# olegiy/manuscript-ocr

Measured on AMD Instinct MI355X. Metric: manuscript pages/sec end-to-end (EAST+TRBA) at 1/2/4/8 MI355X; CER vs CPU ref, higher is better.
Workload: dtype f32 (bf16x3 split operands on the 1x1 / Winograd-domain GEMMs, f32 accumulate)

## Files before the change

### include/msocr.h

```cpp
#ifndef MSOCR_H
#define MSOCR_H
#include <stdint.h>

#ifdef __cplusplus
extern "C" {
#endif

#define MSOCR_F32 0
#define MSOCR_BF16 1

#define MSOCR_OK 0
#define MSOCR_E_ARG (-1)
#define MSOCR_E_LAUNCH (-2)
#define MSOCR_E_NOGPU (-3)

#define MSOCR_CONV_RELU 1u
#define MSOCR_CONV_RESIDUAL 2u
#define MSOCR_CONV_POOL2 4u

typedef struct msocr_conv_desc {
  int32_t dtype;
  int32_t N, H, W, Cin;
  int64_t in_sN, in_sH, in_sW;
  int32_t KH, KW, stride_h, stride_w, pad_h, pad_w;
  int32_t Ho, Wo, Cout;
  int64_t out_ld;
  int64_t res_ld;
  uint32_t flags;
} msocr_conv_desc;

int msocr_conv2d(const msocr_conv_desc* d, const void* in, const void* weight, const float* bias,
                 const void* residual, void* out, void* stream);

#define MSOCR_WINO_2X2 0
#define MSOCR_WINO_4X2 1
#define MSOCR_WINO_4X4 2
int64_t msocr_winograd_workspace_bytes(const msocr_conv_desc* d, int form);
int msocr_winograd_weights_host(int form, const float* w_khwc_host, int Cout, int Cin, float* u_out_host);
int msocr_conv3x3_winograd(const msocr_conv_desc* d, int form, int split, const void* in, const void* u, const float* bias,
                           const void* residual, void* out, void* workspace, void* stream);
int msocr_winograd_input_transform(const msocr_conv_desc* d, int form, const void* in, void* workspace, void* stream);
int msocr_winograd_gemm(const msocr_conv_desc* d, int form, int split, const void* u, void* workspace, void* stream);
int msocr_winograd_output_transform(const msocr_conv_desc* d, int form, const void* workspace, const float* bias, const void* residual,
                                    void* out, void* stream);

int msocr_split_bf16x3_host(const float* w_host, int64_t n, uint16_t* planes_out_host);
int msocr_split_bf16x3_ktile_host(const float* w_host, int64_t nbatch, int64_t rows, int64_t k, uint16_t* planes_out_host);
int msocr_conv1x1_split(const msocr_conv_desc* d, const void* in, const void* weight_planes, const float* bias,
                        const void* residual, void* out, void* stream);
int msocr_conv2d_split(const msocr_conv_desc* d, const void* in, const void* weight_planes, const float* bias,
                       const void* residual, void* out, void* stream);

int64_t msocr_winograd_fused64_workspace_bytes(const msocr_conv_desc* d);
int msocr_conv3x3_winograd_fused64(const msocr_conv_desc* d, int split, const void* in, const void* u, const float* bias,
                                   const void* residual, void* out, void* workspace, void* stream);
int msocr_winograd_fused64_gemm_output(const msocr_conv_desc* d, int split, const void* u, const void* workspace, const float* bias,
                                       const void* residual, void* out, void* stream);

int msocr_normalize_u8(const uint8_t* src, int N, int H, int W, int pad_t, int pad_l, int Hp, int Wp, int cpad,
                       int mode, int dtype, void* out, void* stream);

int msocr_resize_linear_u8(const uint8_t* src, int N, int sh, int sw, uint8_t* dst, int dh, int dw, void* stream);

int msocr_maxpool2d(const void* in, int N, int H, int W, int C, int64_t in_ld, int k, int s, int p, int dtype,
                    void* out, int Ho, int Wo, int64_t out_ld, void* stream);

int msocr_upsample2x_bilinear(const void* in, int N, int H, int W, int C, int64_t in_ld, int dtype, void* out,
                              int64_t out_ld, void* stream);

int msocr_east_head(const void* h1, int64_t npix, int64_t in_ld, int dtype, const float* w9, const float* b9,
                    float* score_out, float* geo_out, void* stream);

int msocr_east_decode(const float* score, const float* geo, int N, int H, int W, float thresh, float scale,
                      int quant, float* cand_out, int32_t* count_out, int max_cand, void* stream);

int64_t msocr_lanms_workspace_bytes(int N, int max_cand);
int msocr_east_lanms(const float* cand, const int32_t* counts, int N, int max_cand, double iou_thr, float* boxes_out,
                     int32_t* nbox_out, void* workspace, void* stream);

int64_t msocr_east_box_tail_workspace_bytes(int N, int max_cand);
int msocr_east_box_tail(const float* boxes, const int32_t* nbox, int N, int max_cand, double expand_w, double expand_h,
                        double scale_x, double scale_y, int axis_aligned_output, int remove_anomalies, double sigma, int min_count,
                        float* out, int32_t* n_out, void* workspace, void* stream);
int msocr_east_box_tail_host(const float* quads_host, int M, double expand_w, double expand_h, double scale_x, double scale_y,
                             int axis_aligned_output, int remove_anomalies, double sigma, int min_count, float* out_host,
                             int32_t* n_out_host);


int msocr_se_residual(const void* x, const void* identity, int N, int HW, int C, int dtype, const float* w1,
                      const float* w2, float* gate_ws, void* out, void* stream);

int msocr_mean_over_h(const void* in, int N, int H, int W, int C, int dtype, float* out, void* stream);

int msocr_bilstm_recurrent(const float* xproj, const float* w_hh_t, int B, int T, int H, float* hcat_out,
                           void* stream);
int msocr_bilstm_recurrent_split(const float* xproj, const uint16_t* whh_planes, int B, int T, int H, float* hcat_out,
                                 void* stream);

typedef struct msocr_attn_weights {
  const float* h2h_wt;
  const float* h2h_b;
  const float* score_w;
  const float* wih_ctx_t;
  const float* wih_tok;
  const float* whh_t;
  const float* b_gates;
  const float* gen_wt;
  const float* gen_b;
} msocr_attn_weights;

int msocr_attn_greedy(const float* batch_H, const float* proj_H, const msocr_attn_weights* w, int B, int T, int H,
                      int V, int steps, int sos_id, int eos_id, int blank_id, float* logits_out, int32_t* ids_out,
                      void* stream);
int64_t msocr_attn_beam_workspace_bytes(int B, int steps, int beam, int V);
int msocr_attn_beam(const float* batch_H, const float* proj_H, const msocr_attn_weights* w, int B, int T, int H,
                    int V, int steps, int beam, const float* lp_dev, float temperature, int sos_id, int eos_id,
                    int blank_id, int32_t* fin_step_out, void* workspace, const int32_t* chunk_id_dev,
                    const int32_t* chunk_size_dev, int32_t* chunk_state_dev, void* stream);
typedef struct msocr_attn_split_weights {
  const uint16_t* h2h_p;
  const uint16_t* whh_p;
  const uint16_t* gen_p;
} msocr_attn_split_weights;

int msocr_attn_beam_hoisted(const float* batch_H, const float* proj_H, const float* ctx_gates, const msocr_attn_weights* w,
                            const msocr_attn_split_weights* ws, int B, int T, int H, int V, int steps, int beam, const float* lp_dev,
                            float temperature, int sos_id, int eos_id, int blank_id, int32_t* fin_step_out, void* workspace,
                            const int32_t* chunk_id_dev, const int32_t* chunk_size_dev, int32_t* chunk_state_dev, void* stream);
int msocr_attn_greedy_hoisted(const float* batch_H, const float* proj_H, const float* ctx_gates, const msocr_attn_weights* w,
                              const msocr_attn_split_weights* ws, int B, int T, int H, int V, int steps, int sos_id, int eos_id,
                              int blank_id, float* logits_out, int32_t* ids_out, void* stream);
int64_t msocr_attn_pack_split_elems(int N);
int msocr_attn_pack_split_host(const float* wt_host, int N, int gate_interleaved, uint16_t* out_host);
int msocr_attn_beam_finalize(const void* workspace, int B, int V, int steps, int beam, const int32_t* trun_dev,
                             float* logits_out, int32_t* ids_out, void* stream);

int msocr_seq_confidence(const float* logits, const int32_t* ids, const int32_t* trun_dev, int B, int V, int steps,
                         float* conf_out, void* stream);

int msocr_crop_resize_pad(const uint8_t* pages, int N, int H, int W, const int32_t* desc_dev,
                          const int32_t* desc_host, int M, int img_h, int img_w, uint8_t* canvases, void* stream);

int msocr_reading_order_host(const int32_t* boxes_host, int n, double y_tol_ratio, double x_gap_ratio,
                             int32_t* order_out_host);

int64_t msocr_reading_order_workspace_bytes(int N, int max_cand);
int msocr_reading_order_crops(const float* boxes, const int32_t* nbox, int N, int max_cand, int page_h, int page_w,
                              int min_text_size, int img_h, int img_w, double y_tol_ratio, double x_gap_ratio, int page_base,
                              int32_t* order_out, int32_t* keep_out, int32_t* desc_out, int32_t* ncrop_out, void* workspace,
                              void* stream);

typedef struct msocr_jpeg_info {
  int32_t width, height, ncomp;
  int32_t hs[3], vs[3];
  int32_t blocks_w[3], blocks_h[3];
  int32_t supported;
  int64_t coef_off[3];
  int64_t coef_total;
  uint16_t quant[3][64];
} msocr_jpeg_info;
int msocr_jpeg_parse_host(const uint8_t* data_host, int64_t len, msocr_jpeg_info* info_out);
int msocr_jpeg_entropy_decode_host(const uint8_t* data_host, int64_t len, const msocr_jpeg_info* info, int16_t* coef_out_host);
int64_t msocr_jpeg_scan_desc_bytes(void);
int64_t msocr_jpeg_scan_prepare_host(const uint8_t* data_host, int64_t len, const msocr_jpeg_info* info, int64_t bytes_base,
                                     void* desc_out, uint32_t* bounds_out, int64_t bounds_cap);
int msocr_jpeg_entropy_decode_device(const uint8_t* bytes_dev, const void* descs_dev, int32_t n_pages, int32_t max_intervals,
                                     const uint32_t* bounds_dev, const int64_t* page_base_dev, int16_t* coef_dev, int64_t coef_total,
                                     int32_t* status_dev, void* stream);
int msocr_jpeg_entropy_decode_intervals_host(const uint8_t* bytes_host, const void* descs_host, int32_t n_pages,
                                             const uint32_t* bounds_host, const int64_t* page_base_host, int16_t* coef_host,
                                             int64_t coef_total, int32_t* status_host);
int64_t msocr_jpeg_workspace_bytes(const msocr_jpeg_info* info);
int msocr_jpeg_reconstruct(const msocr_jpeg_info* info, const int16_t* coef_dev, void* workspace_dev, uint8_t* rgb_out_dev,
                           void* stream);
int msocr_jpeg_reconstruct_host(const msocr_jpeg_info* info, const int16_t* coef_host, uint8_t* rgb_out_host);

int msocr_nchw_f32_to_nhwc(const float* in, int N, int C, int H, int W, int dtype, void* out, int64_t out_ld,
                           void* stream);
int msocr_nhwc_to_nchw_f32(const void* in, int N, int C, int H, int W, int64_t in_ld, int dtype, float* out,
                           void* stream);

const char* msocr_version(void);

#ifdef __cplusplus
}
#endif
#endif
```

### manuscript_ocr_amd/_native.py

```python
import ctypes
import os

import torch

_HERE = os.path.dirname(os.path.abspath(__file__))
LIB_PATH = os.path.join(_HERE, "libmsocr.so")

F32, BF16 = 0, 1
CONV_RELU, CONV_RESIDUAL, CONV_POOL2 = 1, 2, 4
WINO_2X2, WINO_4X2, WINO_4X4 = 0, 1, 2

c_i32, c_i64, c_u32 = ctypes.c_int32, ctypes.c_int64, ctypes.c_uint32
c_f32, c_f64, c_vp = ctypes.c_float, ctypes.c_double, ctypes.c_void_p


class ConvDesc(ctypes.Structure):
    _fields_ = [
        ("dtype", c_i32), ("N", c_i32), ("H", c_i32), ("W", c_i32), ("Cin", c_i32),
        ("in_sN", c_i64), ("in_sH", c_i64), ("in_sW", c_i64),
        ("KH", c_i32), ("KW", c_i32), ("stride_h", c_i32), ("stride_w", c_i32), ("pad_h", c_i32), ("pad_w", c_i32),
        ("Ho", c_i32), ("Wo", c_i32), ("Cout", c_i32),
        ("out_ld", c_i64), ("res_ld", c_i64), ("flags", c_u32),
    ]


class JpegInfo(ctypes.Structure):
    _fields_ = [("width", c_i32), ("height", c_i32), ("ncomp", c_i32), ("hs", c_i32 * 3), ("vs", c_i32 * 3),
                ("blocks_w", c_i32 * 3), ("blocks_h", c_i32 * 3), ("supported", c_i32), ("coef_off", c_i64 * 3),
                ("coef_total", c_i64), ("quant", (ctypes.c_uint16 * 64) * 3)]


class AttnWeights(ctypes.Structure):
    _fields_ = [(n, c_vp) for n in ("h2h_wt", "h2h_b", "score_w", "wih_ctx_t", "wih_tok", "whh_t", "b_gates", "gen_wt", "gen_b")]


class AttnSplitWeights(ctypes.Structure):
    _fields_ = [(n, c_vp) for n in ("h2h_p", "whh_p", "gen_p")]


_SIGS = {
    "msocr_conv2d": (c_i32, [ctypes.POINTER(ConvDesc), c_vp, c_vp, c_vp, c_vp, c_vp, c_vp]),
    "msocr_winograd_workspace_bytes": (c_i64, [ctypes.POINTER(ConvDesc), c_i32]),
    "msocr_winograd_weights_host": (c_i32, [c_i32, c_vp, c_i32, c_i32, c_vp]),
    "msocr_conv3x3_winograd": (c_i32, [ctypes.POINTER(ConvDesc), c_i32, c_i32, c_vp, c_vp, c_vp, c_vp, c_vp, c_vp, c_vp]),
    "msocr_winograd_input_transform": (c_i32, [ctypes.POINTER(ConvDesc), c_i32, c_vp, c_vp, c_vp]),
    "msocr_winograd_gemm": (c_i32, [ctypes.POINTER(ConvDesc), c_i32, c_i32, c_vp, c_vp, c_vp]),
    "msocr_winograd_output_transform": (c_i32, [ctypes.POINTER(ConvDesc), c_i32, c_vp, c_vp, c_vp, c_vp, c_vp]),
    "msocr_winograd_fused64_workspace_bytes": (c_i64, [ctypes.POINTER(ConvDesc)]),
    "msocr_conv3x3_winograd_fused64": (c_i32, [ctypes.POINTER(ConvDesc), c_i32, c_vp, c_vp, c_vp, c_vp, c_vp, c_vp, c_vp]),
    "msocr_winograd_fused64_gemm_output": (c_i32, [ctypes.POINTER(ConvDesc), c_i32, c_vp, c_vp, c_vp, c_vp, c_vp, c_vp]),
    "msocr_split_bf16x3_host": (c_i32, [c_vp, c_i64, c_vp]),
    "msocr_split_bf16x3_ktile_host": (c_i32, [c_vp, c_i64, c_i64, c_i64, c_vp]),
    "msocr_conv1x1_split": (c_i32, [ctypes.POINTER(ConvDesc), c_vp, c_vp, c_vp, c_vp, c_vp, c_vp]),
    "msocr_conv2d_split": (c_i32, [ctypes.POINTER(ConvDesc), c_vp, c_vp, c_vp, c_vp, c_vp, c_vp]),
    "msocr_normalize_u8": (c_i32, [c_vp, c_i32, c_i32, c_i32, c_i32, c_i32, c_i32, c_i32, c_i32, c_i32, c_i32, c_vp, c_vp]),
    "msocr_resize_linear_u8": (c_i32, [c_vp, c_i32, c_i32, c_i32, c_vp, c_i32, c_i32, c_vp]),
    "msocr_maxpool2d": (c_i32, [c_vp, c_i32, c_i32, c_i32, c_i32, c_i64, c_i32, c_i32, c_i32, c_i32, c_vp, c_i32, c_i32, c_i64, c_vp]),
    "msocr_upsample2x_bilinear": (c_i32, [c_vp, c_i32, c_i32, c_i32, c_i32, c_i64, c_i32, c_vp, c_i64, c_vp]),
    "msocr_east_head": (c_i32, [c_vp, c_i64, c_i64, c_i32, c_vp, c_vp, c_vp, c_vp, c_vp]),
    "msocr_east_decode": (c_i32, [c_vp, c_vp, c_i32, c_i32, c_i32, c_f32, c_f32, c_i32, c_vp, c_vp, c_i32, c_vp]),
    "msocr_lanms_workspace_bytes": (c_i64, [c_i32, c_i32]),
    "msocr_east_lanms": (c_i32, [c_vp, c_vp, c_i32, c_i32, c_f64, c_vp, c_vp, c_vp, c_vp]),
    "msocr_se_residual": (c_i32, [c_vp, c_vp, c_i32, c_i32, c_i32, c_i32, c_vp, c_vp, c_vp, c_vp, c_vp]),
    "msocr_mean_over_h": (c_i32, [c_vp, c_i32, c_i32, c_i32, c_i32, c_i32, c_vp, c_vp]),
    "msocr_bilstm_recurrent": (c_i32, [c_vp, c_vp, c_i32, c_i32, c_i32, c_vp, c_vp]),
    "msocr_bilstm_recurrent_split": (c_i32, [c_vp, c_vp, c_i32, c_i32, c_i32, c_vp, c_vp]),
    "msocr_attn_greedy": (c_i32, [c_vp, c_vp, ctypes.POINTER(AttnWeights), c_i32, c_i32, c_i32, c_i32, c_i32, c_i32, c_i32, c_i32,
                                  c_vp, c_vp, c_vp]),
    "msocr_attn_greedy_hoisted": (c_i32, [c_vp, c_vp, c_vp, ctypes.POINTER(AttnWeights), ctypes.POINTER(AttnSplitWeights), c_i32, c_i32,
                                          c_i32, c_i32, c_i32, c_i32, c_i32, c_i32, c_vp, c_vp, c_vp]),
    "msocr_attn_beam": (c_i32, [c_vp, c_vp, ctypes.POINTER(AttnWeights), c_i32, c_i32, c_i32, c_i32, c_i32, c_i32, c_vp, c_f32,
                                c_i32, c_i32, c_i32, c_vp, c_vp, c_vp, c_vp, c_vp, c_vp]),
    "msocr_attn_pack_split_elems": (c_i64, [c_i32]),
    "msocr_attn_pack_split_host": (c_i32, [c_vp, c_i32, c_i32, c_vp]),
    "msocr_attn_beam_hoisted": (c_i32, [c_vp, c_vp, c_vp, ctypes.POINTER(AttnWeights), ctypes.POINTER(AttnSplitWeights), c_i32, c_i32, c_i32, c_i32, c_i32, c_i32, c_vp, c_f32,
                                        c_i32, c_i32, c_i32, c_vp, c_vp, c_vp, c_vp, c_vp, c_vp]),
    "msocr_attn_beam_workspace_bytes": (c_i64, [c_i32, c_i32, c_i32, c_i32]),
    "msocr_attn_beam_finalize": (c_i32, [c_vp, c_i32, c_i32, c_i32, c_i32, c_vp, c_vp, c_vp, c_vp]),
    "msocr_seq_confidence": (c_i32, [c_vp, c_vp, c_vp, c_i32, c_i32, c_i32, c_vp, c_vp]),
    "msocr_crop_resize_pad": (c_i32, [c_vp, c_i32, c_i32, c_i32, c_vp, c_vp, c_i32, c_i32, c_i32, c_vp, c_vp]),
    "msocr_east_box_tail_workspace_bytes": (c_i64, [c_i32, c_i32]),
    "msocr_east_box_tail": (c_i32, [c_vp, c_vp, c_i32, c_i32, c_f64, c_f64, c_f64, c_f64, c_i32, c_i32, c_f64, c_i32, c_vp, c_vp, c_vp, c_vp]),
    "msocr_east_box_tail_host": (c_i32, [c_vp, c_i32, c_f64, c_f64, c_f64, c_f64, c_i32, c_i32, c_f64, c_i32, c_vp, c_vp]),
    "msocr_reading_order_host": (c_i32, [c_vp, c_i32, c_f64, c_f64, c_vp]),
    "msocr_reading_order_workspace_bytes": (c_i64, [c_i32, c_i32]),
    "msocr_reading_order_crops": (c_i32, [c_vp, c_vp, c_i32, c_i32, c_i32, c_i32, c_i32, c_i32, c_i32, c_f64, c_f64, c_i32,
                                          c_vp, c_vp, c_vp, c_vp, c_vp, c_vp]),
    "msocr_jpeg_parse_host": (c_i32, [c_vp, c_i64, ctypes.POINTER(JpegInfo)]),
    "msocr_jpeg_entropy_decode_host": (c_i32, [c_vp, c_i64, ctypes.POINTER(JpegInfo), c_vp]),
    "msocr_jpeg_scan_desc_bytes": (c_i64, []),
    "msocr_jpeg_scan_prepare_host": (c_i64, [c_vp, c_i64, ctypes.POINTER(JpegInfo), c_i64, c_vp, c_vp, c_i64]),
    "msocr_jpeg_entropy_decode_device": (c_i32, [c_vp, c_vp, c_i32, c_i32, c_vp, c_vp, c_vp, c_i64, c_vp, c_vp]),
    "msocr_jpeg_entropy_decode_intervals_host": (c_i32, [c_vp, c_vp, c_i32, c_vp, c_vp, c_vp, c_i64, c_vp]),
    "msocr_jpeg_workspace_bytes": (c_i64, [ctypes.POINTER(JpegInfo)]),
    "msocr_jpeg_reconstruct": (c_i32, [ctypes.POINTER(JpegInfo), c_vp, c_vp, c_vp, c_vp]),
    "msocr_jpeg_reconstruct_host": (c_i32, [ctypes.POINTER(JpegInfo), c_vp, c_vp]),
    "msocr_nchw_f32_to_nhwc": (c_i32, [c_vp, c_i32, c_i32, c_i32, c_i32, c_i32, c_vp, c_i64, c_vp]),
    "msocr_nhwc_to_nchw_f32": (c_i32, [c_vp, c_i32, c_i32, c_i32, c_i32, c_i64, c_i32, c_vp, c_vp]),
    "msocr_version": (ctypes.c_char_p, []),
}

_lib = None


class NativeError(RuntimeError):
    pass


def lib():
    global _lib
    if _lib is None:
        if not os.path.exists(LIB_PATH) and os.path.exists("/opt/rocm/bin/hipcc"):
            import fcntl
            import subprocess
            try:
                with open(os.path.join(_HERE, "csrc", ".build.lock"), "w") as lock:
                    fcntl.flock(lock, fcntl.LOCK_EX)
                    if not os.path.exists(LIB_PATH):
                        subprocess.check_call(["make", "-s", "-j4", "-C", os.path.join(_HERE, "csrc"), "ARCH=gfx950"])
            except Exception as e:
                print(f"[manuscript_ocr_amd] building libmsocr.so failed: {e}")
        if not os.path.exists(LIB_PATH):
            raise NativeError(
                f"{LIB_PATH} not found: build it with `python -c 'import __graft_entry__ as g; g.build()'` "
                "(or `make -C manuscript_ocr_amd/csrc`). There is no CPU fallback."
            )
        L = ctypes.CDLL(LIB_PATH)
        missing = [name for name in _SIGS if not hasattr(L, name)]
        if missing:
            raise NativeError(f"{LIB_PATH} lacks symbols declared in include/msocr.h: {missing}")
        for name, (res, args) in _SIGS.items():
            fn = getattr(L, name)
            fn.restype, fn.argtypes = res, args
        _lib = L
    return _lib


def exported_symbols():
    return list(_SIGS)


def check(rc, what):
    if rc != 0:
        raise NativeError(f"{what} failed with code {rc} (-1 bad argument/shape, -2 launch failure)")
```

### manuscript_ocr_amd/csrc/winograd.hip

```cpp
#include <hip/hip_runtime.h>
#include <stdint.h>

#include "internal.h"
#include "msocr.h"

#define MSOCR_LAUNCH(...) do { (void)hipGetLastError(); hipLaunchKernelGGL(__VA_ARGS__); } while (0)

typedef float f32x4 __attribute__((ext_vector_type(4)));

template <int M> __device__ void wino_bt1(const f32x4 d[M + 2], f32x4 r[M + 2]);
template <int M> __device__ void wino_at1(const f32x4 m[M + 2], f32x4 y[M]);

template <> __device__ __forceinline__ void wino_bt1<2>(const f32x4 d[4], f32x4 r[4]) {
  r[0] = d[0] - d[2];
  r[1] = d[1] + d[2];
  r[2] = d[2] - d[1];
  r[3] = d[1] - d[3];
}
template <> __device__ __forceinline__ void wino_at1<2>(const f32x4 m[4], f32x4 y[2]) {
  y[0] = (m[0] + m[1]) + m[2];
  y[1] = (m[1] - m[2]) - m[3];
}

__device__ __forceinline__ void wino44_bt(const f32x4 d[6], f32x4 r[6]) {
  constexpr float k97_36 = 97.0f / 36.0f, k4_9 = 4.0f / 9.0f, k9_4 = 2.25f, k3_2 = 1.5f, k2_3 = 2.0f / 3.0f;
#pragma unroll
  for (int e = 0; e < 4; ++e) {
    r[0][e] = fmaf(-k97_36, d[2][e], d[0][e]) + d[4][e];
    r[5][e] = fmaf(-k97_36, d[3][e], d[1][e]) + d[5][e];
    const float e1 = fmaf(-k4_9, d[2][e], d[4][e]), o1 = fmaf(k3_2, d[3][e], -k2_3 * d[1][e]);
    const float e2 = fmaf(-k9_4, d[2][e], d[4][e]), o2 = fmaf(k2_3, d[3][e], -k3_2 * d[1][e]);
    r[1][e] = e1 + o1; r[2][e] = e1 - o1;
    r[3][e] = e2 + o2; r[4][e] = e2 - o2;
  }
}
__device__ __forceinline__ void wino44_at(const f32x4 m[6], f32x4 y[4]) {
  constexpr float k3_2 = 1.5f, k2_3 = 2.0f / 3.0f, k9_4 = 2.25f, k4_9 = 4.0f / 9.0f, k27_8 = 3.375f, k8_27 = 8.0f / 27.0f;
#pragma unroll
  for (int e = 0; e < 4; ++e) {
    const float p12 = m[1][e] + m[2][e], d12 = m[1][e] - m[2][e], p34 = m[3][e] + m[4][e], d34 = m[3][e] - m[4][e];
    y[0][e] = (m[0][e] + p12) + p34;
    y[1][e] = fmaf(k3_2, d12, k2_3 * d34);
    y[2][e] = fmaf(k9_4, p12, k4_9 * p34);
    y[3][e] = fmaf(k27_8, d12, k8_27 * d34) + m[5][e];
  }
}
template <> __device__ __forceinline__ void wino_bt1<4>(const f32x4 d[6], f32x4 r[6]) { wino44_bt(d, r); }
template <> __device__ __forceinline__ void wino_at1<4>(const f32x4 m[6], f32x4 y[4]) { wino44_at(m, y); }


struct WinoGeom {
  int N, H, W;
  int TH, TW;
  long Mt;
};

template <int MH, int MW>
__device__ __forceinline__ void wino_input_body(const float* in, long sN, long sH, long sW, int C, WinoGeom g, float* V) {
  constexpr int PH = MH + 2, PW = MW + 2;
  constexpr bool w_first = MH == 4;
  const int cch = C >> 2;
  const long gid = (long)blockIdx.x * 256 + threadIdx.x;
  const long t = gid / cch;
  const int c = (int)(gid - t * cch) << 2;
  if (t >= g.Mt) return;
  const int tw = (int)(t % g.TW);
  const long r = t / g.TW;
  const int th = (int)(r % g.TH);
  const int n = (int)(r / g.TH);
  const int h0 = MH * th - 1, w0 = MW * tw - 1;
  const float* base = in + (long)n * sN + c;
  f32x4 q[PH][PW];
#pragma unroll
  for (int i = 0; i < PH; ++i) {
    const int hi = h0 + i;
    const bool okh = (unsigned)hi < (unsigned)g.H;
    f32x4 d[PW];
#pragma unroll
    for (int j = 0; j < PW; ++j) {
      const int wi = w0 + j;
      const bool ok = okh && (unsigned)wi < (unsigned)g.W;
      const f32x4 v = *reinterpret_cast<const f32x4*>(ok ? base + (long)hi * sH + (long)wi * sW : base);
      d[j] = ok ? v : (f32x4){0.f, 0.f, 0.f, 0.f};
    }
    if constexpr (w_first) {
      wino_bt1<MW>(d, q[i]);
    } else {
#pragma unroll
      for (int j = 0; j < PW; ++j) q[i][j] = d[j];
    }
  }
  const long plane = g.Mt * (long)C;
  float* o = V + t * (long)C + c;
  if constexpr (w_first) {
#pragma unroll
    for (int j = 0; j < PW; ++j) {
      f32x4 col[PH], v[PH];
#pragma unroll
      for (int i = 0; i < PH; ++i) col[i] = q[i][j];
      wino_bt1<MH>(col, v);
#pragma unroll
      for (int i = 0; i < PH; ++i) *reinterpret_cast<f32x4*>(o + (i * PW + j) * plane) = v[i];
    }
  } else {
#pragma unroll
    for (int i = 0; i < PH; ++i) {
      f32x4 row[PW], v[PW];
#pragma unroll
      for (int j = 0; j < PW; ++j) {
        f32x4 col[PH], hv[PH];
#pragma unroll
        for (int k = 0; k < PH; ++k) col[k] = q[k][j];
        wino_bt1<MH>(col, hv);
        row[j] = hv[i];
      }
      wino_bt1<MW>(row, v);
#pragma unroll
      for (int j = 0; j < PW; ++j) *reinterpret_cast<f32x4*>(o + (i * PW + j) * plane) = v[j];
    }
  }
}

template <int MH, int MW>
__device__ __forceinline__ void wino_output_body(const float* Mw, int Cout, WinoGeom g, const float* bias, const float* res, long res_ld,
                                                 int relu, float* out, long out_ld) {
  constexpr int PH = MH + 2, PW = MW + 2;
  const int cch = Cout >> 2;
  const long gid = (long)blockIdx.x * 256 + threadIdx.x;
  const long t = gid / cch;
  const int c = (int)(gid - t * cch) << 2;
  if (t >= g.Mt) return;
  const int tw = (int)(t % g.TW);
  const long r = t / g.TW;
  const int th = (int)(r % g.TH);
  const int n = (int)(r / g.TH);
  const long plane = g.Mt * (long)Cout;
  const float* mp = Mw + t * (long)Cout + c;
  f32x4 mt[PH][PW];
  if constexpr (MH == 2) {
#pragma unroll
    for (int i = 0; i < PH; ++i)
#pragma unroll
      for (int j = 0; j < PW; ++j) mt[i][j] = *reinterpret_cast<const f32x4*>(mp + (i * PW + j) * plane);
  }
  f32x4 s[MH][PW];
#pragma unroll
  for (int j = 0; j < PW; ++j) {
    f32x4 m[PH], y[MH];
#pragma unroll
    for (int i = 0; i < PH; ++i) m[i] = MH == 2 ? mt[i][j] : *reinterpret_cast<const f32x4*>(mp + (i * PW + j) * plane);
    wino_at1<MH>(m, y);
#pragma unroll
    for (int a = 0; a < MH; ++a) s[a][j] = y[a];
  }
  f32x4 b = {0.f, 0.f, 0.f, 0.f};
  if (bias) b = *reinterpret_cast<const f32x4*>(bias + c);
#pragma unroll
  for (int a = 0; a < MH; ++a) {
    const int ho = MH * th + a;
    if (ho >= g.H) continue;
    f32x4 y[MW];
    wino_at1<MW>(s[a], y);
#pragma unroll
    for (int j = 0; j < MW; ++j) {
      const int wo = MW * tw + j;
      if (wo >= g.W) continue;
      const long pix = ((long)n * g.H + ho) * g.W + wo;
      f32x4 v = y[j] + b;
      if (res) v += *reinterpret_cast<const f32x4*>(res + pix * res_ld + c);
      if (relu) {
        v[0] = fmaxf(v[0], 0.f); v[1] = fmaxf(v[1], 0.f); v[2] = fmaxf(v[2], 0.f); v[3] = fmaxf(v[3], 0.f);
      }
      *reinterpret_cast<f32x4*>(out + pix * out_ld + c) = v;
    }
  }
}

#define WINO_TRANSFORM_KERNELS(PREFIX, MH, MW)                                                                                    \
  __global__ __launch_bounds__(256) void PREFIX##_input_kernel(const float* __restrict__ in, long sN, long sH, long sW, int C,   \
                                                               WinoGeom g, float* __restrict__ V) {                            \
    wino_input_body<MH, MW>(in, sN, sH, sW, C, g, V);                                                                            \
  }                                                                                                                              \
  __global__ __launch_bounds__(256) void PREFIX##_output_kernel(const float* __restrict__ Mw, int Cout, WinoGeom g,              \
                                                                const float* __restrict__ bias, const float* __restrict__ res,  \
                                                                long res_ld, int relu, float* __restrict__ out, long out_ld) {  \
    wino_output_body<MH, MW>(Mw, Cout, g, bias, res, res_ld, relu, out, out_ld);                                                 \
  }
WINO_TRANSFORM_KERNELS(wino, 2, 2)
WINO_TRANSFORM_KERNELS(wino42, 4, 2)
WINO_TRANSFORM_KERNELS(wino44, 4, 4)
#undef WINO_TRANSFORM_KERNELS

static const int kWinoTile[3][2] = {{2, 2}, {4, 2}, {4, 4}};

static int wino_points(int form) { return (kWinoTile[form][0] + 2) * (kWinoTile[form][1] + 2); }

static bool wino_geom(const msocr_conv_desc* d, int form, WinoGeom* g) {
  if (form < MSOCR_WINO_2X2 || form > MSOCR_WINO_4X4 || !d || d->dtype != MSOCR_F32) return false;
  if (d->KH != 3 || d->KW != 3 || d->stride_h != 1 || d->stride_w != 1 || d->pad_h != 1 || d->pad_w != 1) return false;
  if (d->N <= 0 || d->H <= 0 || d->W <= 0 || d->Ho != d->H || d->Wo != d->W) return false;
  if (d->Cin <= 0 || d->Cin % 16 || d->Cout <= 0 || d->Cout % 32) return false;
  if ((long)d->N * ((d->H + 1) / 2) * ((d->W + 1) / 2) > 0x7fffffffL) return false;
  const int mh = kWinoTile[form][0], mw = kWinoTile[form][1];
  g->N = d->N; g->H = d->H; g->W = d->W;
  g->TH = (d->H + mh - 1) / mh; g->TW = (d->W + mw - 1) / mw;
  g->Mt = (long)d->N * g->TH * g->TW;
  return wino_points(form) * g->Mt * (long)(d->Cin > d->Cout ? d->Cin : d->Cout) <= 0x3fffffffffffL;
}

static bool wino_strides_ok(const msocr_conv_desc* d) { return !(d->in_sN % 4 || d->in_sH % 4 || d->in_sW % 4); }

static int wino_check(const msocr_conv_desc* d, int form, WinoGeom* g) {
  if (!wino_geom(d, form, g) || !wino_strides_ok(d) || d->out_ld % 4 || d->out_ld < d->Cout) return MSOCR_E_ARG;
  return MSOCR_OK;
}

static bool wino_gemm_ok(int form, int split) {
  if (split != 0 && split != 1) return false;
  return form == MSOCR_WINO_4X2 || (form == MSOCR_WINO_2X2 && !split) || (form == MSOCR_WINO_4X4 && split);
}

extern "C" int64_t msocr_winograd_workspace_bytes(const msocr_conv_desc* d, int form) {
  WinoGeom g;
  if (!wino_geom(d, form, &g)) return -1;
  return wino_points(form) * g.Mt * ((int64_t)d->Cin + d->Cout) * (int64_t)sizeof(float);
}

static int wino_launch_input(const msocr_conv_desc* d, int form, const WinoGeom& g, const void* in, void* workspace, void* stream) {
  if (!in || !workspace || (((uintptr_t)in | (uintptr_t)workspace) & 15)) return MSOCR_E_ARG;
  const long nb_in = (g.Mt * (d->Cin / 4) + 255) / 256;
  if (nb_in > 0x7fffffffL) return MSOCR_E_ARG;
  const dim3 grid((unsigned)nb_in), blk(256);
  hipStream_t st = (hipStream_t)stream;
  const float* x = (const float*)in;
  float* V = (float*)workspace;
  if (form == MSOCR_WINO_2X2) MSOCR_LAUNCH(wino_input_kernel, grid, blk, 0, st, x, (long)d->in_sN, (long)d->in_sH, (long)d->in_sW, d->Cin, g, V);
  else if (form == MSOCR_WINO_4X2) MSOCR_LAUNCH(wino42_input_kernel, grid, blk, 0, st, x, (long)d->in_sN, (long)d->in_sH, (long)d->in_sW, d->Cin, g, V);
  else MSOCR_LAUNCH(wino44_input_kernel, grid, blk, 0, st, x, (long)d->in_sN, (long)d->in_sH, (long)d->in_sW, d->Cin, g, V);
  return hipGetLastError() == hipSuccess ? MSOCR_OK : MSOCR_E_LAUNCH;
}

extern "C" int msocr_winograd_input_transform(const msocr_conv_desc* d, int form, const void* in, void* workspace, void* stream) {
  WinoGeom g;
  if (wino_check(d, form, &g) != MSOCR_OK) return MSOCR_E_ARG;
  return wino_launch_input(d, form, g, in, workspace, stream);
}

extern "C" int msocr_winograd_gemm(const msocr_conv_desc* d, int form, int split, const void* u, void* workspace, void* stream) {
  WinoGeom g;
  if (!wino_gemm_ok(form, split) || wino_check(d, form, &g) != MSOCR_OK || !u || !workspace) return MSOCR_E_ARG;
  if (split && (d->Cin % 32 || d->Cout % 64)) return MSOCR_E_ARG;
  const int P = wino_points(form);
  float* V = (float*)workspace;
  float* Mw = V + P * g.Mt * (long)d->Cin;
  if (split) return msocr_internal_gemm_split_batched(V, (const uint16_t*)u, Mw, g.Mt, d->Cout, d->Cin, P, (hipStream_t)stream);
  return msocr_internal_gemm_f32_batched(V, (const float*)u, Mw, g.Mt, d->Cout, d->Cin, P, (hipStream_t)stream);
}

extern "C" int msocr_winograd_output_transform(const msocr_conv_desc* d, int form, const void* workspace, const float* bias,
                                               const void* residual, void* out, void* stream) {
  WinoGeom g;
  if (wino_check(d, form, &g) != MSOCR_OK || !out || !workspace) return MSOCR_E_ARG;
  if (((uintptr_t)out | (uintptr_t)workspace) & 15) return MSOCR_E_ARG;
  const bool has_res = (d->flags & MSOCR_CONV_RESIDUAL) != 0;
  if (has_res && (!residual || d->res_ld % 4 || d->res_ld < d->Cout || ((uintptr_t)residual & 15))) return MSOCR_E_ARG;
  if (bias && ((uintptr_t)bias & 15)) return MSOCR_E_ARG;
  const long nb_out = (g.Mt * (d->Cout / 4) + 255) / 256;
  if (nb_out > 0x7fffffffL) return MSOCR_E_ARG;
  const float* Mw = (const float*)workspace + wino_points(form) * g.Mt * (long)d->Cin;
  const float* rp = has_res ? (const float*)residual : nullptr;
  const int relu = (d->flags & MSOCR_CONV_RELU) ? 1 : 0;
  const dim3 grid((unsigned)nb_out), blk(256);
  hipStream_t st = (hipStream_t)stream;
  float* o = (float*)out;
  if (form == MSOCR_WINO_2X2) MSOCR_LAUNCH(wino_output_kernel, grid, blk, 0, st, Mw, d->Cout, g, bias, rp, (long)d->res_ld, relu, o, (long)d->out_ld);
  else if (form == MSOCR_WINO_4X2) MSOCR_LAUNCH(wino42_output_kernel, grid, blk, 0, st, Mw, d->Cout, g, bias, rp, (long)d->res_ld, relu, o, (long)d->out_ld);
  else MSOCR_LAUNCH(wino44_output_kernel, grid, blk, 0, st, Mw, d->Cout, g, bias, rp, (long)d->res_ld, relu, o, (long)d->out_ld);
  return hipGetLastError() == hipSuccess ? MSOCR_OK : MSOCR_E_LAUNCH;
}

extern "C" int msocr_conv3x3_winograd(const msocr_conv_desc* d, int form, int split, const void* in, const void* u, const float* bias,
                                      const void* residual, void* out, void* workspace, void* stream) {
  if (!u || !wino_gemm_ok(form, split)) return MSOCR_E_ARG;
  int rc = msocr_winograd_input_transform(d, form, in, workspace, stream);
  if (rc != MSOCR_OK) return rc;
  rc = msocr_winograd_gemm(d, form, split, u, workspace, stream);
  if (rc != MSOCR_OK) return rc;
  return msocr_winograd_output_transform(d, form, workspace, bias, residual, out, stream);
}

typedef unsigned int u32x4w __attribute__((ext_vector_type(4)));
#ifndef WINO_FUSED_PFD
#define WINO_FUSED_PFD 3
#endif

typedef __bf16 bf16x8w __attribute__((ext_vector_type(8)));
typedef unsigned int u32x2w __attribute__((ext_vector_type(2)));
__device__ __forceinline__ unsigned int wino_split_step(float& x, float& y) {
  typedef __bf16 bf16x2 __attribute__((ext_vector_type(2)));
  typedef float f32x2 __attribute__((ext_vector_type(2)));
  const f32x2 v = {x, y};
  const bf16x2 h = __builtin_convertvector(v, bf16x2);
  const unsigned int pk = __builtin_bit_cast(unsigned int, h);
  x -= __uint_as_float(pk << 16);
  y -= __uint_as_float(pk & 0xffff0000u);
  return pk;
}

template <bool POOL, bool SPLIT = false>
__global__ __launch_bounds__(256, 3) void wino42_fused64_kernel(const float* __restrict__ V, const void* __restrict__ Uv, int Cout,
                                                                 WinoGeom g, const float* __restrict__ bias,
                                                                 const float* __restrict__ res, long res_ld, int relu,
                                                                 float* __restrict__ out, long out_ld) {
  constexpr int K = 64, BM = 32, BN = 32, ROWB = K * 4;
  constexpr int ROWS = 128, PLANE = BM * ROWS;
  constexpr int STAGE_BYTES = SPLIT ? 6 * PLANE : (BM + BN) * ROWB;
  __shared__ __attribute__((aligned(16))) unsigned char smem[2][STAGE_BYTES];
  const int tid = threadIdx.x, lane = tid & 63, wave = tid >> 6;
  const int mi = wave >> 1, nj = wave & 1;
  const int r16 = lane & 15, kg = lane >> 4;
  const int nbn = Cout / BN;
  const long nblk = (long)gridDim.x;
  long bid = blockIdx.x;
  {
    const long q = nblk >> 3, r = nblk & 7, x = bid & 7;
    bid = (x < r ? x * (q + 1) : r * (q + 1) + (x - r) * q) + (bid >> 3);
  }
  const int nb = (int)(bid % nbn);
  const long m0 = (bid / nbn) * BM;
  const int n0 = nb * BN;
  f32x4 acc[24];

  if constexpr (SPLIT) {
    const unsigned short* U = reinterpret_cast<const unsigned short*>(Uv);
    const int chunk = tid & 15, row0 = tid >> 4;
    const int bchunk = tid & 7, brow = tid >> 3;
    const long planeV = g.Mt * (long)K, planeU = (long)Cout * K, uplane = 24 * planeU;
    const float* pa[2];
#pragma unroll
    for (int i = 0; i < 2; ++i) {
      long m = m0 + row0 + 16 * i;
      if (m >= g.Mt) m = g.Mt - 1;
      pa[i] = V + m * K + chunk * 4;
    }
    const unsigned short* pb = U + (long)(n0 + brow) * K + bchunk * 8;
    constexpr int PFD = 2;
    u32x4w ra[PFD][2], rb[PFD][3];
    auto gload = [&](int p) {
#pragma unroll
      for (int i = 0; i < 2; ++i) ra[p % PFD][i] = *reinterpret_cast<const u32x4w*>(pa[i] + p * planeV);
#pragma unroll
      for (int pl = 0; pl < 3; ++pl) rb[p % PFD][pl] = *reinterpret_cast<const u32x4w*>(pb + pl * uplane + p * planeU);
    };
    auto sstore = [&](int p) {
      unsigned char* st = &smem[p & 1][0];
#pragma unroll
      for (int i = 0; i < 2; ++i) {
        const int row = row0 + 16 * i;
        float x0 = __uint_as_float(ra[p % PFD][i][0]), x1 = __uint_as_float(ra[p % PFD][i][1]);
        float x2 = __uint_as_float(ra[p % PFD][i][2]), x3 = __uint_as_float(ra[p % PFD][i][3]);
        unsigned char* dst = st + row * ROWS + (((chunk >> 1) ^ (row & 7)) << 4) + ((chunk & 1) << 3);
#pragma unroll
        for (int pl = 0; pl < 3; ++pl) {
          u32x2w v;
          v[0] = wino_split_step(x0, x1);
          v[1] = wino_split_step(x2, x3);
          *reinterpret_cast<u32x2w*>(dst + pl * PLANE) = v;
        }
      }
#pragma unroll
      for (int pl = 0; pl < 3; ++pl)
        *reinterpret_cast<u32x4w*>(st + (3 + pl) * PLANE + brow * ROWS + ((bchunk ^ (brow & 7)) << 4)) = rb[p % PFD][pl];
    };
#pragma unroll
    for (int q = 0; q < PFD; ++q) gload(q);
    sstore(0);
    __syncthreads();
#pragma unroll
    for (int p = 0; p < 24; ++p) {
      if (p + PFD < 24) gload(p + PFD);
      const unsigned char* st = &smem[p & 1][0];
      const int rowa = mi * 16 + r16, rowb = nj * 16 + r16;
      f32x4 c4 = {0.f, 0.f, 0.f, 0.f};
#pragma unroll
      for (int ks = 0; ks < 2; ++ks) {
        const int c = 4 * ks + kg;
        bf16x8w fa[3], fb[3];
#pragma unroll
        for (int pl = 0; pl < 3; ++pl) {
          fa[pl] = *reinterpret_cast<const bf16x8w*>(st + pl * PLANE + rowa * ROWS + ((c ^ (rowa & 7)) << 4));
          fb[pl] = *reinterpret_cast<const bf16x8w*>(st + (3 + pl) * PLANE + rowb * ROWS + ((c ^ (rowb & 7)) << 4));
        }
        c4 = __builtin_amdgcn_mfma_f32_16x16x32_bf16(fa[2], fb[0], c4, 0, 0, 0);
        c4 = __builtin_amdgcn_mfma_f32_16x16x32_bf16(fa[0], fb[2], c4, 0, 0, 0);
        c4 = __builtin_amdgcn_mfma_f32_16x16x32_bf16(fa[1], fb[1], c4, 0, 0, 0);
        c4 = __builtin_amdgcn_mfma_f32_16x16x32_bf16(fa[1], fb[0], c4, 0, 0, 0);
        c4 = __builtin_amdgcn_mfma_f32_16x16x32_bf16(fa[0], fb[1], c4, 0, 0, 0);
        c4 = __builtin_amdgcn_mfma_f32_16x16x32_bf16(fa[0], fb[0], c4, 0, 0, 0);
      }
      acc[p] = c4;
      if (p + 1 < 24) sstore(p + 1);
      __syncthreads();
    }
  } else {
  const float* U = reinterpret_cast<const float*>(Uv);
  const int chunk = tid & 15, row0 = tid >> 4;
  const long planeV = g.Mt * (long)K, planeU = (long)Cout * K;
  const float* pa[2];
  const float* pb[2];
#pragma unroll
  for (int i = 0; i < 2; ++i) {
    long m = m0 + row0 + 16 * i;
    if (m >= g.Mt) m = g.Mt - 1;
    pa[i] = V + m * K + chunk * 4;
    pb[i] = U + (long)(n0 + row0 + 16 * i) * K + chunk * 4;
  }
  constexpr int PFD = WINO_FUSED_PFD;
  u32x4w ra[PFD][2], rb[PFD][2];
  auto gload = [&](int p) {
#pragma unroll
    for (int i = 0; i < 2; ++i) {
      ra[p % PFD][i] = *reinterpret_cast<const u32x4w*>(pa[i] + p * planeV);
      rb[p % PFD][i] = *reinterpret_cast<const u32x4w*>(pb[i] + p * planeU);
    }
  };
  auto sstore = [&](int p) {
#pragma unroll
    for (int i = 0; i < 2; ++i) {
      const int row = row0 + 16 * i;
      *reinterpret_cast<u32x4w*>(&smem[p & 1][row * ROWB + ((chunk ^ (row & 15)) << 4)]) = ra[p % PFD][i];
      *reinterpret_cast<u32x4w*>(&smem[p & 1][(BM + row) * ROWB + ((chunk ^ (row & 15)) << 4)]) = rb[p % PFD][i];
    }
  };
#pragma unroll
  for (int q = 0; q < PFD; ++q) gload(q);
  sstore(0);
  __syncthreads();
#pragma unroll
  for (int p = 0; p < 24; ++p) {
    if (p + PFD < 24) gload(p + PFD);
    const unsigned char* sa = &smem[p & 1][0];
    const unsigned char* sb = sa + BM * ROWB;
    const int rowa = mi * 16 + r16, rowb = nj * 16 + r16;
    u32x4w fa[4], fb[4];
#pragma unroll
    for (int q = 0; q < 4; ++q) {
      const int c = kg * 4 + q;
      fa[q] = *reinterpret_cast<const u32x4w*>(sa + rowa * ROWB + ((c ^ (rowa & 15)) << 4));
      fb[q] = *reinterpret_cast<const u32x4w*>(sb + rowb * ROWB + ((c ^ (rowb & 15)) << 4));
    }
    f32x4 c4 = {0.f, 0.f, 0.f, 0.f};
#pragma unroll
    for (int q = 0; q < 4; ++q)
#pragma unroll
      for (int e = 0; e < 4; ++e)
        c4 = __builtin_amdgcn_mfma_f32_16x16x4f32(__uint_as_float(fa[q][e]), __uint_as_float(fb[q][e]), c4, 0, 0, 0);
    acc[p] = c4;
    if (p + 1 < 24) sstore(p + 1);
    __syncthreads();
  }

  }

  const int co = n0 + nj * 16 + r16;
  const float b = bias ? bias[co] : 0.f;
#pragma unroll
  for (int e = 0; e < 4; ++e) {
    const long t = m0 + mi * 16 + 4 * kg + e;
    if (t >= g.Mt) continue;
    const int tw = (int)(t % g.TW);
    const long r = t / g.TW;
    const int th = (int)(r % g.TH);
    const int n = (int)(r / g.TH);
    float s[4][4];
#pragma unroll
    for (int j = 0; j < 4; ++j) {
      const float m0_ = acc[0 * 4 + j][e], m1 = acc[1 * 4 + j][e], m2 = acc[2 * 4 + j][e], m3 = acc[3 * 4 + j][e], m4 = acc[4 * 4 + j][e],
                  m5 = acc[5 * 4 + j][e];
      const float p12 = m1 + m2, d12 = m1 - m2, p34 = m3 + m4, d34 = m3 - m4;
      s[0][j] = (m0_ + p12) + p34;
      s[1][j] = fmaf(1.5f, d12, (2.0f / 3.0f) * d34);
      s[2][j] = fmaf(2.25f, p12, (4.0f / 9.0f) * p34);
      s[3][j] = fmaf(3.375f, d12, (8.0f / 27.0f) * d34) + m5;
    }
    float y[4][2];
#pragma unroll
    for (int i = 0; i < 4; ++i) {
      y[i][0] = ((s[i][0] + s[i][1]) + s[i][2]) + b;
      y[i][1] = ((s[i][1] - s[i][2]) - s[i][3]) + b;
    }
    if constexpr (POOL) {
      const int Hp = g.H >> 1, Wp = g.W >> 1;
#pragma unroll
      for (int i2 = 0; i2 < 2; ++i2) {
        const int hp = 2 * th + i2;
        if (hp >= Hp || tw >= Wp) continue;
        float v0 = y[2 * i2][0], v1 = y[2 * i2][1], v2 = y[2 * i2 + 1][0], v3 = y[2 * i2 + 1][1];
        if (relu) { v0 = fmaxf(v0, 0.f); v1 = fmaxf(v1, 0.f); v2 = fmaxf(v2, 0.f); v3 = fmaxf(v3, 0.f); }
        out[(((long)n * Hp + hp) * Wp + tw) * out_ld + co] = fmaxf(fmaxf(v0, v1), fmaxf(v2, v3));
      }
    } else {
#pragma unroll
      for (int i = 0; i < 4; ++i) {
        const int ho = 4 * th + i;
        if (ho >= g.H) continue;
#pragma unroll
        for (int j = 0; j < 2; ++j) {
          const int wo = 2 * tw + j;
          if (wo >= g.W) continue;
          const long pix = ((long)n * g.H + ho) * g.W + wo;
          float v = y[i][j];
          if (res) v += res[pix * res_ld + co];
          if (relu) v = fmaxf(v, 0.f);
          out[pix * out_ld + co] = v;
        }
      }
    }
  }
}

template <bool POOL>
__global__ __launch_bounds__(256, 2) void wino42_fused64_v2_kernel(const float* __restrict__ V, const unsigned short* __restrict__ U, int Cout,
                                                                    WinoGeom g, const float* __restrict__ bias,
                                                                    const float* __restrict__ res, long res_ld, int relu,
                                                                    float* __restrict__ out, long out_ld) {
  constexpr int K = 64, BM = 64, BN = 64, ROWS = 128, PLANE = BM * ROWS;
  typedef float f32x16w __attribute__((ext_vector_type(16)));
  __shared__ __attribute__((aligned(16))) unsigned char smem[6 * PLANE];
  const int tid = threadIdx.x, lane = tid & 63, wave = tid >> 6;
  const int wm = wave >> 1, wn = wave & 1;
  const int r32 = lane & 31, half = lane >> 5;
  const int nbn = Cout / BN;
  const long nblk = (long)gridDim.x;
  long bid = blockIdx.x;
  {
    const long q = nblk >> 3, r = nblk & 7, x = bid & 7;
    bid = (x < r ? x * (q + 1) : r * (q + 1) + (x - r) * q) + (bid >> 3);
  }
  const int nb = (int)(bid % nbn);
  const long m0 = (bid / nbn) * BM;
  const int n0 = nb * BN;

  const int chunk = tid & 15, row0 = tid >> 4;
  const int bchunk = tid & 7, brow = tid >> 3;
  const long planeV = g.Mt * (long)K, planeU = (long)Cout * K, uplane = 24 * planeU;
  const float* pa[4];
#pragma unroll
  for (int i = 0; i < 4; ++i) {
    long m = m0 + row0 + 16 * i;
    if (m >= g.Mt) m = g.Mt - 1;
    pa[i] = V + m * K + chunk * 4;
  }
  const unsigned short* pb = U + (long)(n0 + brow) * K + bchunk * 8;
  u32x4w ra[4], rb[3][2];
  auto gload = [&](int p) {
#pragma unroll
    for (int i = 0; i < 4; ++i) ra[i] = *reinterpret_cast<const u32x4w*>(pa[i] + p * planeV);
#pragma unroll
    for (int pl = 0; pl < 3; ++pl)
#pragma unroll
      for (int j = 0; j < 2; ++j) rb[pl][j] = *reinterpret_cast<const u32x4w*>(pb + pl * uplane + p * planeU + (long)j * 32 * K);
  };
  auto sstore = [&]() {
#pragma unroll
    for (int i = 0; i < 4; ++i) {
      const int row = row0 + 16 * i;
      float x0 = __uint_as_float(ra[i][0]), x1 = __uint_as_float(ra[i][1]), x2 = __uint_as_float(ra[i][2]), x3 = __uint_as_float(ra[i][3]);
      unsigned char* dst = smem + row * ROWS + (((chunk >> 1) ^ (row & 7)) << 4) + ((chunk & 1) << 3);
#pragma unroll
      for (int pl = 0; pl < 3; ++pl) {
        u32x2w v;
        v[0] = wino_split_step(x0, x1);
        v[1] = wino_split_step(x2, x3);
        *reinterpret_cast<u32x2w*>(dst + pl * PLANE) = v;
      }
    }
#pragma unroll
    for (int pl = 0; pl < 3; ++pl)
#pragma unroll
      for (int j = 0; j < 2; ++j) {
        const int row = brow + 32 * j;
        *reinterpret_cast<u32x4w*>(smem + (3 + pl) * PLANE + row * ROWS + ((bchunk ^ (row & 7)) << 4)) = rb[pl][j];
      }
  };

  f32x16w Y[8];
#pragma unroll
  for (int o = 0; o < 8; ++o)
#pragma unroll
    for (int e = 0; e < 16; ++e) Y[o][e] = 0.f;

  gload(0);
  sstore();
  __syncthreads();
  __shared__ float s_cf[24][8];
  if (tid < 192) {
    const float t6[4][6] = {{1, 1, 1, 1, 1, 0}, {0, 1.5f, -1.5f, 2.0f / 3.0f, -2.0f / 3.0f, 0}, {0, 2.25f, 2.25f, 4.0f / 9.0f, 4.0f / 9.0f, 0},
                            {0, 3.375f, -3.375f, 8.0f / 27.0f, -8.0f / 27.0f, 1}};
    const float t4[2][4] = {{1, 1, 1, 0}, {0, 1, -1, -1}};
    const int pp = tid >> 3, o = tid & 7;
    s_cf[pp][o] = t6[o >> 1][pp >> 2] * t4[o & 1][pp & 3];
  }
  __syncthreads();
  const int rowa = wm * 32 + r32, rowb = wn * 32 + r32;
#pragma unroll 1
  for (int p = 0; p < 24; ++p) {
    if (p + 1 < 24) gload(p + 1);
    f32x16w m;
#pragma unroll
    for (int e = 0; e < 16; ++e) m[e] = 0.f;
#pragma unroll
    for (int ks = 0; ks < 4; ++ks) {
      const int c = 2 * ks + half;
      bf16x8w fa[3], fb[3];
#pragma unroll
      for (int pl = 0; pl < 3; ++pl) {
        fa[pl] = *reinterpret_cast<const bf16x8w*>(smem + pl * PLANE + rowa * ROWS + ((c ^ (rowa & 7)) << 4));
        fb[pl] = *reinterpret_cast<const bf16x8w*>(smem + (3 + pl) * PLANE + rowb * ROWS + ((c ^ (rowb & 7)) << 4));
      }
      m = __builtin_amdgcn_mfma_f32_32x32x16_bf16(fa[2], fb[0], m, 0, 0, 0);
      m = __builtin_amdgcn_mfma_f32_32x32x16_bf16(fa[0], fb[2], m, 0, 0, 0);
      m = __builtin_amdgcn_mfma_f32_32x32x16_bf16(fa[1], fb[1], m, 0, 0, 0);
      m = __builtin_amdgcn_mfma_f32_32x32x16_bf16(fa[1], fb[0], m, 0, 0, 0);
      m = __builtin_amdgcn_mfma_f32_32x32x16_bf16(fa[0], fb[1], m, 0, 0, 0);
      m = __builtin_amdgcn_mfma_f32_32x32x16_bf16(fa[0], fb[0], m, 0, 0, 0);
    }
#pragma unroll
    for (int o = 0; o < 8; ++o) {
      const float cf = s_cf[p][o];
#pragma unroll
      for (int e = 0; e < 16; ++e) Y[o][e] = fmaf(cf, m[e], Y[o][e]);
    }
    __syncthreads();
    if (p + 1 < 24) sstore();
    __syncthreads();
  }

  const int co = n0 + wn * 32 + r32;
  const float bv = bias ? bias[co] : 0.f;
#pragma unroll
  for (int e = 0; e < 16; ++e) {
    const long t = m0 + wm * 32 + (e & 3) + 8 * (e >> 2) + 4 * half;
    if (t >= g.Mt) continue;
    const int tw = (int)(t % g.TW);
    const long r = t / g.TW;
    const int th = (int)(r % g.TH);
    const int n = (int)(r / g.TH);
    if constexpr (POOL) {
      const int Hp = g.H >> 1, Wp = g.W >> 1;
#pragma unroll
      for (int i2 = 0; i2 < 2; ++i2) {
        const int hp = 2 * th + i2;
        if (hp >= Hp || tw >= Wp) continue;
        float v0 = Y[4 * i2 + 0][e] + bv, v1 = Y[4 * i2 + 1][e] + bv, v2 = Y[4 * i2 + 2][e] + bv, v3 = Y[4 * i2 + 3][e] + bv;
        if (relu) { v0 = fmaxf(v0, 0.f); v1 = fmaxf(v1, 0.f); v2 = fmaxf(v2, 0.f); v3 = fmaxf(v3, 0.f); }
        out[(((long)n * Hp + hp) * Wp + tw) * out_ld + co] = fmaxf(fmaxf(v0, v1), fmaxf(v2, v3));
      }
    } else {
#pragma unroll
      for (int a = 0; a < 4; ++a) {
        const int ho = 4 * th + a;
        if (ho >= g.H) continue;
#pragma unroll
        for (int b = 0; b < 2; ++b) {
          const int wo = 2 * tw + b;
          if (wo >= g.W) continue;
          const long pix = ((long)n * g.H + ho) * g.W + wo;
          float v = Y[a * 2 + b][e] + bv;
          if (res) v += res[pix * res_ld + co];
          if (relu) v = fmaxf(v, 0.f);
          out[pix * out_ld + co] = v;
        }
      }
    }
  }
}

static int wino_fused64_check(const msocr_conv_desc* d, WinoGeom* g) {
  if (!wino_geom(d, MSOCR_WINO_4X2, g) || d->Cin != 64 || !wino_strides_ok(d) || d->out_ld < d->Cout) return MSOCR_E_ARG;
  if (d->flags & MSOCR_CONV_POOL2) {
    if ((d->H & 1) || (d->W & 1) || (d->flags & MSOCR_CONV_RESIDUAL)) return MSOCR_E_ARG;
  }
  return MSOCR_OK;
}

extern "C" int64_t msocr_winograd_fused64_workspace_bytes(const msocr_conv_desc* d) {
  WinoGeom g;
  if (wino_fused64_check(d, &g) != MSOCR_OK) return -1;
  return 24 * g.Mt * (int64_t)d->Cin * (int64_t)sizeof(float);
}

extern "C" int msocr_winograd_fused64_gemm_output(const msocr_conv_desc* d, int split, const void* u, const void* workspace,
                                                  const float* bias, const void* residual, void* out, void* stream) {
  WinoGeom g;
  if ((split != 0 && split != 1) || wino_fused64_check(d, &g) != MSOCR_OK || !u || !workspace || !out) return MSOCR_E_ARG;
  if (((uintptr_t)workspace | (uintptr_t)u) & 15) return MSOCR_E_ARG;
  const bool has_res = (d->flags & MSOCR_CONV_RESIDUAL) != 0;
  if (has_res && (!residual || d->res_ld < d->Cout)) return MSOCR_E_ARG;
  const long nblk = ((g.Mt + 31) / 32) * (long)(d->Cout / 32);
  if (nblk <= 0 || nblk > 0x7fffffffL) return MSOCR_E_ARG;
  const int relu = (d->flags & MSOCR_CONV_RELU) ? 1 : 0;
  const float* rp = has_res ? (const float*)residual : nullptr;
  const dim3 grid((unsigned)nblk), blk(256);
  hipStream_t st = (hipStream_t)stream;
  const float* ws = (const float*)workspace;
  static const bool v2 = !(getenv("MSOCR_WINO_FUSED_V2") && getenv("MSOCR_WINO_FUSED_V2")[0] == '0');
  if (split && v2 && d->Cout % 64 == 0) {
    const long nblk2 = ((g.Mt + 63) / 64) * (long)(d->Cout / 64);
    if (nblk2 <= 0 || nblk2 > 0x7fffffffL) return MSOCR_E_ARG;
    const dim3 grid2((unsigned)nblk2);
    const unsigned short* up = (const unsigned short*)u;
    if (d->flags & MSOCR_CONV_POOL2)
      MSOCR_LAUNCH((wino42_fused64_v2_kernel<true>), grid2, blk, 0, st, ws, up, d->Cout, g, bias, (const float*)nullptr, 0L, relu, (float*)out, (long)d->out_ld);
    else
      MSOCR_LAUNCH((wino42_fused64_v2_kernel<false>), grid2, blk, 0, st, ws, up, d->Cout, g, bias, rp, (long)d->res_ld, relu, (float*)out, (long)d->out_ld);
    return hipGetLastError() == hipSuccess ? MSOCR_OK : MSOCR_E_LAUNCH;
  }
  if (d->flags & MSOCR_CONV_POOL2) {
    if (split) MSOCR_LAUNCH((wino42_fused64_kernel<true, true>), grid, blk, 0, st, ws, u, d->Cout, g, bias, (const float*)nullptr, 0L, relu, (float*)out, (long)d->out_ld);
    else MSOCR_LAUNCH((wino42_fused64_kernel<true, false>), grid, blk, 0, st, ws, u, d->Cout, g, bias, (const float*)nullptr, 0L, relu, (float*)out, (long)d->out_ld);
  } else {
    if (split) MSOCR_LAUNCH((wino42_fused64_kernel<false, true>), grid, blk, 0, st, ws, u, d->Cout, g, bias, rp, (long)d->res_ld, relu, (float*)out, (long)d->out_ld);
    else MSOCR_LAUNCH((wino42_fused64_kernel<false, false>), grid, blk, 0, st, ws, u, d->Cout, g, bias, rp, (long)d->res_ld, relu, (float*)out, (long)d->out_ld);
  }
  return hipGetLastError() == hipSuccess ? MSOCR_OK : MSOCR_E_LAUNCH;
}

extern "C" int msocr_conv3x3_winograd_fused64(const msocr_conv_desc* d, int split, const void* in, const void* u, const float* bias,
                                              const void* residual, void* out, void* workspace, void* stream) {
  WinoGeom g;
  if ((split != 0 && split != 1) || wino_fused64_check(d, &g) != MSOCR_OK || !u) return MSOCR_E_ARG;
  const int rc = wino_launch_input(d, MSOCR_WINO_4X2, g, in, workspace, stream);
  if (rc != MSOCR_OK) return rc;
  return msocr_winograd_fused64_gemm_output(d, split, u, workspace, bias, residual, out, stream);
}

extern "C" int msocr_winograd_weights_host(int form, const float* w_khwc, int Cout, int Cin, float* u_out) {
  if (form < MSOCR_WINO_2X2 || form > MSOCR_WINO_4X4 || !w_khwc || !u_out || Cout <= 0 || Cin <= 0) return MSOCR_E_ARG;
  static const double G4[4][3] = {{1.0, 0.0, 0.0}, {0.5, 0.5, 0.5}, {0.5, -0.5, 0.5}, {0.0, 0.0, 1.0}};
  static const double G6[6][3] = {{1.0, 0.0, 0.0},
                                  {8.0 / 65, 12.0 / 65, 18.0 / 65},     {8.0 / 65, -12.0 / 65, 18.0 / 65},
                                  {-81.0 / 130, -27.0 / 65, -18.0 / 65}, {-81.0 / 130, 27.0 / 65, -18.0 / 65},
                                  {0.0, 0.0, 1.0}};
  const int PH = kWinoTile[form][0] + 2, PW = kWinoTile[form][1] + 2;
  const double(*Gh)[3] = PH == 6 ? G6 : G4;
  const double(*Gw)[3] = PW == 6 ? G6 : G4;
  const long plane = (long)Cout * Cin;
  for (int co = 0; co < Cout; ++co) {
    const float* w = w_khwc + (long)co * 9 * Cin;
    for (int c = 0; c < Cin; ++c) {
      double gw[6][3];
      for (int xi = 0; xi < PH; ++xi)
        for (int kw = 0; kw < 3; ++kw)
          gw[xi][kw] = Gh[xi][0] * w[(0 * 3 + kw) * Cin + c] + Gh[xi][1] * w[(1 * 3 + kw) * Cin + c] + Gh[xi][2] * w[(2 * 3 + kw) * Cin + c];
      for (int xi = 0; xi < PH; ++xi)
        for (int nu = 0; nu < PW; ++nu)
          u_out[(xi * PW + nu) * plane + (long)co * Cin + c] =
              (float)(gw[xi][0] * Gw[nu][0] + gw[xi][1] * Gw[nu][1] + gw[xi][2] * Gw[nu][2]);
    }
  }
  return MSOCR_OK;
}
```

### manuscript_ocr_amd/ops.py

```python
import ctypes
import os

import torch

from . import _native as nat


PROFILE = None


def _prof_begin():
    if PROFILE is None:
        return None
    e0 = torch.cuda.Event(enable_timing=True)
    e0.record()
    return e0


def _prof_end(e0, kind, work, tag=None):
    if e0 is None or PROFILE is None:
        return
    e1 = torch.cuda.Event(enable_timing=True)
    e1.record()
    PROFILE.append((e0, e1, kind, work, tag))


def _dt(t):
    if t.dtype == torch.float32:
        return nat.F32
    if t.dtype == torch.bfloat16:
        return nat.BF16
    raise TypeError(f"unsupported dtype {t.dtype}")


def _stream():
    return ctypes.c_void_p(torch.cuda.current_stream().cuda_stream)


def _need_cuda(*ts):
    for t in ts:
        if t is not None and not t.is_cuda:
            raise nat.NativeError("native ops need device tensors (no CPU fallback)")


def _pixel_dense_ld(t):
    N, H, W, C = t.shape
    ld = t.stride(2)
    if t.stride(3) != 1 or t.stride(1) != W * ld or (N > 1 and t.stride(0) != H * W * ld) or ld < C:
        raise ValueError(f"tensor is not pixel-dense NHWC: shape {tuple(t.shape)} strides {t.stride()}")
    return ld


WINOGRAD_MIN_CIN = int(os.environ.get("MSOCR_WINOGRAD_MIN_CIN", "128"))


WINO_WS_LIMIT = int(os.environ.get("MSOCR_WINO_WS_LIMIT", str(1 << 30)))
_WINO_ARENA = {}


def _wino_workspace(nbytes, device):
    if torch.cuda.is_current_stream_capturing():
        return torch.empty((nbytes,), dtype=torch.uint8, device=device)
    key = (device.index, torch.cuda.current_stream().cuda_stream)
    buf = _WINO_ARENA.get(key)
    if buf is None or buf.numel() < nbytes:
        buf = None
        _WINO_ARENA.pop(key, None)
        buf = torch.empty((nbytes,), dtype=torch.uint8, device=device)
        _WINO_ARENA[key] = buf
    return buf


WINOGRAD_TALL = int(os.environ.get("MSOCR_WINO_TALL", "1"))


def _tall_pays(H):
    return 24 * (-(-H // 4)) < 16 * (-(-H // 2))


WINOGRAD_SQUARE = int(os.environ.get("MSOCR_WINO_SQUARE", "1"))
WINOGRAD_SQUARE_MIN_CIN = int(os.environ.get("MSOCR_WINO_SQUARE_MIN_CIN", "512"))


def _square_pays(W):
    return 36 * (-(-W // 4)) < 24 * (-(-W // 2))


WINO_FORMS = {nat.WINO_2X2: ("winograd", 16, (2, 2)), nat.WINO_4X2: ("winograd42", 24, (4, 2)), nat.WINO_4X4: ("winograd44", 36, (4, 4))}


def _wino_weights(wh, form):
    Cout, _, _, Cin = wh.shape
    u = torch.empty((WINO_FORMS[form][1], Cout, Cin), dtype=torch.float32)
    nat.check(nat.lib().msocr_winograd_weights_host(form, wh.data_ptr(), Cout, Cin, u.data_ptr()), "winograd_weights_host")
    return u


WINOGRAD_FUSED64 = int(os.environ.get("MSOCR_WINO_FUSED64", "1"))


SPLIT_BF16X3 = int(os.environ.get("MSOCR_SPLIT", "1"))


def split_planes(t):
    th = t.detach().float().cpu().contiguous()
    planes = torch.empty((3,) + tuple(th.shape), dtype=torch.int16)
    nat.check(nat.lib().msocr_split_bf16x3_host(th.data_ptr(), th.numel(), planes.data_ptr()), "split_bf16x3_host")
    return planes.view(torch.bfloat16).to(t.device)


def split_planes_ktile(t, nbatch, rows):
    th = t.detach().float().cpu().contiguous()
    k = th.numel() // (nbatch * rows)
    assert k % 32 == 0 and nbatch * rows * k == th.numel()
    planes = torch.empty((3, nbatch, k // 32, rows, 32), dtype=torch.int16)
    nat.check(nat.lib().msocr_split_bf16x3_ktile_host(th.data_ptr(), nbatch, rows, k, planes.data_ptr()), "split_bf16x3_ktile_host")
    return planes.view(torch.bfloat16).to(t.device)


def unsplit_planes_ktile(planes):
    nb, kt, rows = planes.shape[1:4]
    return planes.float().sum(0).permute(0, 2, 1, 3).reshape(nb, rows, kt * 32)


SPLIT_MIN_K = int(os.environ.get("MSOCR_SPLIT_MIN_K", "128"))


def _split_eligible(w):
    Cout, KH, KW, Cin = w.shape
    return w.dtype == torch.float32 and Cin % 32 == 0 and Cout % 64 == 0 and KH * KW * Cin >= SPLIT_MIN_K


def attach_split(w, split=None):
    if split is False:
        w._msocr_nosplit = True
        return w
    Cout, KH, KW, Cin = w.shape
    if (SPLIT_BF16X3 if split is None else split) and KH == 1 and KW == 1 and _split_eligible(w):
        w._msocr_split = split_planes_ktile(w, 1, Cout)
    return w


def attach_winograd(w, split=None, square=True):
    Cout, KH, KW, Cin = w.shape
    if (WINOGRAD_MIN_CIN and WINOGRAD_FUSED64 and WINOGRAD_TALL and w.dtype == torch.float32 and KH == 3 and KW == 3 and Cin == 64
            and Cin < WINOGRAD_MIN_CIN and Cout % 32 == 0):
        u42 = _wino_weights(w.detach().cpu().contiguous(), nat.WINO_4X2)
        w._msocr_wino42_fused = u42.to(w.device)
        v2 = os.environ.get("MSOCR_WINO_FUSED_V2", "1") != "0"
        if (SPLIT_BF16X3 if split is None else split) and ((v2 and Cout % 64 == 0) or Cout >= 128):
            w._msocr_wino42_fused_split = split_planes(u42).to(w.device)
        return w
    if not (WINOGRAD_MIN_CIN and w.dtype == torch.float32 and KH == 3 and KW == 3 and Cin >= WINOGRAD_MIN_CIN and Cin % 16 == 0
            and Cout % 32 == 0):
        return w
    wh = w.detach().cpu().contiguous()
    w._msocr_wino = _wino_weights(wh, nat.WINO_2X2).to(w.device)
    u42 = _wino_weights(wh, nat.WINO_4X2)
    w._msocr_wino42 = u42.to(w.device)
    if (SPLIT_BF16X3 if split is None else split) and Cin % 32 == 0 and Cout % 64 == 0:
        w._msocr_wino42_split = split_planes_ktile(u42, 24, Cout).to(w.device)
        if WINOGRAD_SQUARE and square and Cin >= WINOGRAD_SQUARE_MIN_CIN:
            w._msocr_wino44_split = split_planes_ktile(_wino_weights(wh, nat.WINO_4X4), 36, Cout).to(w.device)
    return w


def _winograd(d, x, w, u, form, split, bias, residual, out, alg, fused=False, pool2=False):
    N, H, W, Cin = x.shape
    Cout = w.shape[0]
    stem, npts, (mh, mw) = WINO_FORMS[form]
    name = stem + ("_fused" if fused else "") + ("_split" if split else "")
    L = nat.lib()
    nbytes = L.msocr_winograd_fused64_workspace_bytes(ctypes.byref(d)) if fused else L.msocr_winograd_workspace_bytes(ctypes.byref(d), form)
    if nbytes < 0:
        raise nat.NativeError(f"{name}: unsupported shape {tuple(x.shape)} * {tuple(w.shape)} pool2={pool2}")
    parts = min(N, -(-nbytes // WINO_WS_LIMIT))
    per = -(-N // parts)
    ws = _wino_workspace(nbytes if parts == 1 else (nbytes // N) * per, x.device)
    bp = bias.data_ptr() if bias is not None else None
    what = f"msocr_conv3x3_{name} {tuple(x.shape)} * {tuple(w.shape)}"
    TH, TW = -(-H // mh), -(-W // mw)
    out_px = H * W // (4 if pool2 else 1)
    res_io = 2 if residual is not None else 1
    for n0 in range(0, N, per):
        n1 = min(N, n0 + per)
        d.N = n1 - n0
        xp, rp, op = x[n0:n1].data_ptr(), (residual[n0:n1].data_ptr() if residual is not None else None), out[n0:n1].data_ptr()
        if PROFILE is None:
            if fused:
                rc = L.msocr_conv3x3_winograd_fused64(ctypes.byref(d), int(split), xp, u.data_ptr(), bp, rp, op, ws.data_ptr(), _stream())
            else:
                rc = L.msocr_conv3x3_winograd(ctypes.byref(d), form, int(split), xp, u.data_ptr(), bp, rp, op, ws.data_ptr(), _stream())
            nat.check(rc, what)
            continue
        nn, mt = n1 - n0, (n1 - n0) * TH * TW
        e = _prof_begin()
        nat.check(L.msocr_winograd_input_transform(ctypes.byref(d), form, xp, ws.data_ptr(), _stream()), what)
        _prof_end(e, "wino_in", 4.0 * (nn * H * W * Cin + npts * mt * Cin), (mt, Cin))
        e = _prof_begin()
        if fused:
            rc = L.msocr_winograd_fused64_gemm_output(ctypes.byref(d), int(split), u.data_ptr(), ws.data_ptr(), bp, rp, op, _stream())
        else:
            rc = L.msocr_winograd_gemm(ctypes.byref(d), form, int(split), u.data_ptr(), ws.data_ptr(), _stream())
        nat.check(rc, what)
        io = x.element_size() * (nn * H * W * Cin + nn * out_px * Cout * res_io + Cout * 9 * Cin)
        _prof_end(e, "conv_gemm", (alg * nn / N, 2.0 * npts * mt * Cin * Cout, io), (nn * H * W, Cout, 9 * Cin, name))
        if not fused:
            e = _prof_begin()
            nat.check(L.msocr_winograd_output_transform(ctypes.byref(d), form, ws.data_ptr(), bp, rp, op, _stream()), what)
            _prof_end(e, "wino_out", 4.0 * (npts * mt * Cout + nn * H * W * Cout * res_io), (mt, Cout))
    d.N = N


def conv2d(x, w, bias, stride=(1, 1), pad=(0, 0), relu=False, residual=None, out=None, out_hw=None, alg_k=None, pool2=False):
    _need_cuda(x, w, bias, residual, out)
    N, H, W, Cin = x.shape
    Cout, KH, KW, Cw = w.shape
    assert Cw == Cin and w.is_contiguous() and w.dtype == x.dtype and x.stride(3) == 1
    sh, sw = stride
    ph, pw = pad
    Ho, Wo = out_hw if out_hw else ((H + 2 * ph - KH) // sh + 1, (W + 2 * pw - KW) // sw + 1)
    wino = (sh, sw, ph, pw) == (1, 1, 1, 1) and (Ho, Wo) == (H, W)
    fused = (getattr(w, "_msocr_wino42_fused", None) is not None and WINOGRAD_FUSED64 and WINOGRAD_TALL and wino and _tall_pays(H)
             and (not pool2 or (H % 2 == 0 and W % 2 == 0 and residual is None)))
    if pool2 and not fused:
        return maxpool2d(conv2d(x, w, bias, stride, pad, relu, residual, None, out_hw, alg_k), 2, 2, 0, out=out)
    u = getattr(w, "_msocr_wino", None)
    use_wino = u is not None and wino
    oh, ow = (Ho // 2, Wo // 2) if pool2 else (Ho, Wo)
    if out is None:
        out = torch.empty((N, oh, ow, Cout), dtype=x.dtype, device=x.device)
    assert out.shape == (N, oh, ow, Cout) and out.dtype == x.dtype
    d = nat.ConvDesc()
    d.dtype = _dt(x)
    d.N, d.H, d.W, d.Cin = N, H, W, Cin
    d.in_sN, d.in_sH, d.in_sW = x.stride(0), x.stride(1), x.stride(2)
    d.KH, d.KW, d.stride_h, d.stride_w, d.pad_h, d.pad_w = KH, KW, sh, sw, ph, pw
    d.Ho, d.Wo, d.Cout = Ho, Wo, Cout
    d.out_ld = _pixel_dense_ld(out)
    flags = (nat.CONV_RELU if relu else 0) | (nat.CONV_POOL2 if pool2 else 0)
    rp = None
    if residual is not None:
        assert residual.shape == out.shape and residual.dtype == x.dtype
        d.res_ld = _pixel_dense_ld(residual)
        flags |= nat.CONV_RESIDUAL
        rp = residual.data_ptr()
    d.flags = flags
    if bias is not None:
        assert bias.dtype == torch.float32 and bias.numel() == Cout and bias.is_contiguous()
    bp = bias.data_ptr() if bias is not None else None
    alg = 2.0 * N * Ho * Wo * Cout * (alg_k if alg_k else KH * KW * Cin)
    if fused:
        up = getattr(w, "_msocr_wino42_fused_split", None) if SPLIT_BF16X3 else None
        u = w._msocr_wino42_fused if up is None else up
        _winograd(d, x, w, u, nat.WINO_4X2, up is not None, bias, residual, out, alg, fused=True, pool2=pool2)
    elif use_wino:
        form, split = nat.WINO_2X2, False
        if WINOGRAD_TALL and _tall_pays(H) and getattr(w, "_msocr_wino42", None) is not None:
            form, u = nat.WINO_4X2, w._msocr_wino42
            up = getattr(w, "_msocr_wino42_split", None)
            if up is not None and SPLIT_BF16X3:
                u, split = up, True
            up44 = getattr(w, "_msocr_wino44_split", None)
            if up44 is not None and SPLIT_BF16X3 and WINOGRAD_SQUARE and _square_pays(W):
                form, u, split = nat.WINO_4X4, up44, True
        _winograd(d, x, w, u, form, split, bias, residual, out, alg)
    else:
        wp = getattr(w, "_msocr_split", None)
        if (wp is None and SPLIT_BF16X3 and not getattr(w, "_msocr_nosplit", False) and _split_eligible(w)
                and not torch.cuda.is_current_stream_capturing()):
            wp = w._msocr_split = split_planes_ktile(w, 1, Cout)
        split = wp is not None and SPLIT_BF16X3 and KH * KW * Cin >= SPLIT_MIN_K and all(v % 4 == 0 for v in x.stride()[:3])
        lean = (split and (KH, KW, sh, sw, ph, pw) == (1, 1, 1, 1, 0, 0) and (Ho, Wo) == (H, W)
                and (H == 1 or x.stride(1) == W * x.stride(2)) and (N == 1 or x.stride(0) == H * W * x.stride(2)))
        e = _prof_begin()
        if split:
            fn = nat.lib().msocr_conv1x1_split if lean else nat.lib().msocr_conv2d_split
            rc = fn(ctypes.byref(d), x.data_ptr(), wp.data_ptr(), bp, rp, out.data_ptr(), _stream())
            nat.check(rc, f"msocr_conv{'1x1' if lean else '2d'}_split {tuple(x.shape)} * {tuple(w.shape)}")
        else:
            rc = nat.lib().msocr_conv2d(ctypes.byref(d), x.data_ptr(), w.data_ptr(), bp, rp, out.data_ptr(), _stream())
            nat.check(rc, f"msocr_conv2d {tuple(x.shape)} * {tuple(w.shape)}")
        io = x.element_size() * (N * H * W * Cin + N * Ho * Wo * Cout * (2 if residual is not None else 1) + Cout * KH * KW * Cin)
        _prof_end(e, "conv_gemm", (alg, 2.0 * N * Ho * Wo * Cout * KH * KW * Cin, io),
                  (N * Ho * Wo, Cout, KH * KW * Cin, "direct_split" if split else "direct"))
    return out


def normalize_u8(imgs_u8, pad_t, pad_l, Hp, Wp, mode, dtype, cpad=4):
    _need_cuda(imgs_u8)
    N, H, W, C = imgs_u8.shape
    assert C == 3 and imgs_u8.dtype == torch.uint8 and imgs_u8.is_contiguous()
    out = torch.empty((N, Hp, Wp, cpad), dtype=dtype, device=imgs_u8.device)
    nat.check(nat.lib().msocr_normalize_u8(imgs_u8.data_ptr(), N, H, W, pad_t, pad_l, Hp, Wp, cpad, mode, _dt(out), out.data_ptr(),
                                           _stream()),
              "normalize_u8")
    return out


def resize_linear_u8(src, dh, dw):
    _need_cuda(src)
    N, sh, sw, C = src.shape
    assert C == 3 and src.dtype == torch.uint8 and src.is_contiguous()
    dst = torch.empty((N, dh, dw, 3), dtype=torch.uint8, device=src.device)
    nat.check(nat.lib().msocr_resize_linear_u8(src.data_ptr(), N, sh, sw, dst.data_ptr(), dh, dw, _stream()), "resize_linear_u8")
    return dst


def maxpool2d(x, k, s, p, out=None):
    _need_cuda(x, out)
    N, H, W, C = x.shape
    Ho, Wo = (H + 2 * p - k) // s + 1, (W + 2 * p - k) // s + 1
    if out is None:
        out = torch.empty((N, Ho, Wo, C), dtype=x.dtype, device=x.device)
    e = _prof_begin()
    nat.check(nat.lib().msocr_maxpool2d(x.data_ptr(), N, H, W, C, _pixel_dense_ld(x), k, s, p, _dt(x), out.data_ptr(), Ho, Wo,
                                        _pixel_dense_ld(out), _stream()), "maxpool2d")
    _prof_end(e, "maxpool", float(x.element_size()) * N * C * (H * W + Ho * Wo))
    return out


def upsample2x_into(x, out):
    _need_cuda(x, out)
    N, H, W, C = x.shape
    assert out.shape[0] == N and out.shape[1] == 2 * H and out.shape[2] == 2 * W and out.dtype == x.dtype
    nat.check(nat.lib().msocr_upsample2x_bilinear(x.data_ptr(), N, H, W, C, _pixel_dense_ld(x), _dt(x), out.data_ptr(),
                                                  _pixel_dense_ld(out), _stream()), "upsample2x")
    return out


def east_head(h1, w9, b9, score=None, geo=None):
    _need_cuda(h1, w9, b9)
    N, H, W, C = h1.shape
    assert C == 32 and w9.shape == (9, 32) and w9.dtype == torch.float32
    if score is None:
        score = torch.empty((N, H, W), dtype=torch.float32, device=h1.device)
    if geo is None:
        geo = torch.empty((N, H, W, 8), dtype=torch.float32, device=h1.device)
    nat.check(nat.lib().msocr_east_head(h1.data_ptr(), N * H * W, _pixel_dense_ld(h1), _dt(h1), w9.data_ptr(), b9.data_ptr(),
                                        score.data_ptr(), geo.data_ptr(), _stream()), "east_head")
    return score, geo


def east_decode(score, geo, thresh, scale, quant, max_cand):
    _need_cuda(score, geo)
    N, H, W = score.shape
    assert score.dtype == torch.float32 and geo.shape == (N, H, W, 8) and score.is_contiguous() and geo.is_contiguous()
    cand = torch.empty((N, max_cand, 9), dtype=torch.float32, device=score.device)
    counts = torch.empty((N,), dtype=torch.int32, device=score.device)
    nat.check(nat.lib().msocr_east_decode(score.data_ptr(), geo.data_ptr(), N, H, W, float(thresh), float(scale), int(quant),
                                          cand.data_ptr(), counts.data_ptr(), max_cand, _stream()), "east_decode")
    return cand, counts


def east_lanms(cand, counts, iou_thr, workspace=None):
    _need_cuda(cand, counts)
    N, max_cand, _ = cand.shape
    if workspace is None:
        nbytes = nat.lib().msocr_lanms_workspace_bytes(N, max_cand)
        workspace = torch.empty((nbytes,), dtype=torch.uint8, device=cand.device)
    boxes = torch.empty_like(cand)
    nbox = torch.empty((N,), dtype=torch.int32, device=cand.device)
    nat.check(nat.lib().msocr_east_lanms(cand.data_ptr(), counts.data_ptr(), N, max_cand, float(iou_thr), boxes.data_ptr(),
                                         nbox.data_ptr(), workspace.data_ptr(), _stream()), "east_lanms")
    return boxes, nbox


def east_box_tail(boxes, nbox, expand_w, expand_h, scale_x, scale_y, axis_aligned, remove_anomalies, sigma, min_count):
    _need_cuda(boxes, nbox)
    N, max_cand, _ = boxes.shape
    ws = torch.empty((nat.lib().msocr_east_box_tail_workspace_bytes(N, max_cand),), dtype=torch.uint8, device=boxes.device)
    out = torch.empty_like(boxes)
    n_out = torch.empty((N,), dtype=torch.int32, device=boxes.device)
    nat.check(nat.lib().msocr_east_box_tail(boxes.data_ptr(), nbox.data_ptr(), N, max_cand, float(expand_w), float(expand_h),
                                            float(scale_x), float(scale_y), int(bool(axis_aligned)), int(bool(remove_anomalies)),
                                            float(sigma), int(min_count), out.data_ptr(), n_out.data_ptr(), ws.data_ptr(), _stream()),
              "east_box_tail")
    return out, n_out


def reading_order_crops(boxes, nbox, page_hw, min_text_size, img_h, img_w, page_base=0, y_tol_ratio=0.6, x_gap_ratio=float("inf")):
    _need_cuda(boxes, nbox)
    N, max_cand, _ = boxes.shape
    dev = boxes.device
    ws = torch.empty((nat.lib().msocr_reading_order_workspace_bytes(N, max_cand),), dtype=torch.uint8, device=dev)
    order = torch.empty((N, max_cand), dtype=torch.int32, device=dev)
    keep = torch.empty((N, max_cand), dtype=torch.int32, device=dev)
    desc = torch.empty((N, max_cand, 8), dtype=torch.int32, device=dev)
    ncrop = torch.empty((N,), dtype=torch.int32, device=dev)
    nat.check(nat.lib().msocr_reading_order_crops(boxes.data_ptr(), nbox.data_ptr(), N, max_cand, int(page_hw[0]), int(page_hw[1]),
                                                  int(min_text_size), int(img_h), int(img_w), float(y_tol_ratio), float(x_gap_ratio),
                                                  int(page_base), order.data_ptr(), keep.data_ptr(), desc.data_ptr(), ncrop.data_ptr(),
                                                  ws.data_ptr(), _stream()), "reading_order_crops")
    return order, keep, desc, ncrop


def nchw_to_nhwc(x_f32, dtype, out=None):
    _need_cuda(x_f32)
    N, C, H, W = x_f32.shape
    assert x_f32.dtype == torch.float32 and x_f32.is_contiguous()
    if out is None:
        out = torch.empty((N, H, W, C), dtype=dtype, device=x_f32.device)
    nat.check(nat.lib().msocr_nchw_f32_to_nhwc(x_f32.data_ptr(), N, C, H, W, _dt(out), out.data_ptr(), _pixel_dense_ld(out), _stream()),
              "nchw_to_nhwc")
    return out


def nhwc_to_nchw_f32(x):
    _need_cuda(x)
    N, H, W, C = x.shape
    out = torch.empty((N, C, H, W), dtype=torch.float32, device=x.device)
    nat.check(nat.lib().msocr_nhwc_to_nchw_f32(x.data_ptr(), N, C, H, W, _pixel_dense_ld(x), _dt(x), out.data_ptr(), _stream()),
              "nhwc_to_nchw")
    return out


def se_residual(x, identity, w1, w2, out=None):
    _need_cuda(x, identity, w1, w2)
    N, H, W, C = x.shape
    assert x.is_contiguous() and identity.is_contiguous() and identity.shape == x.shape and identity.dtype == x.dtype
    assert w1.shape == (C // 16, C) and w2.shape == (C, C // 16) and w1.dtype == torch.float32
    if out is None:
        out = torch.empty_like(x)
    gate = torch.empty((N, C), dtype=torch.float32, device=x.device)
    e = _prof_begin()
    nat.check(nat.lib().msocr_se_residual(x.data_ptr(), identity.data_ptr(), N, H * W, C, _dt(x), w1.data_ptr(), w2.data_ptr(),
                                          gate.data_ptr(), out.data_ptr(), _stream()), "se_residual")
    _prof_end(e, "se_residual", 3.0 * x.element_size() * N * H * W * C, (N, H * W, C))
    return out


def mean_over_h(x):
    _need_cuda(x)
    N, H, W, C = x.shape
    assert x.is_contiguous()
    out = torch.empty((N, W, C), dtype=torch.float32, device=x.device)
    nat.check(nat.lib().msocr_mean_over_h(x.data_ptr(), N, H, W, C, _dt(x), out.data_ptr(), _stream()), "mean_over_h")
    return out


def bilstm_recurrent(xproj, whh_t, B, T, H, whh_planes=None):
    _need_cuda(xproj, whh_t)
    assert xproj.is_contiguous() and xproj.numel() == B * T * 8 * H and whh_t.shape == (2, H, H, 4) and whh_t.is_contiguous()
    out = torch.empty((B, T, 2 * H), dtype=torch.float32, device=xproj.device)
    e = _prof_begin()
    if (whh_planes is not None and H == 256 and SPLIT_BF16X3 and B * T * 8 * H < 2 ** 32
            and os.environ.get("MSOCR_BILSTM_MFMA", "1") != "0"):
        nat.check(nat.lib().msocr_bilstm_recurrent_split(xproj.data_ptr(), whh_planes.data_ptr(), B, T, H, out.data_ptr(), _stream()),
                  "bilstm_recurrent_split")
    else:
        nat.check(nat.lib().msocr_bilstm_recurrent(xproj.data_ptr(), whh_t.data_ptr(), B, T, H, out.data_ptr(), _stream()), "bilstm_recurrent")
    _prof_end(e, "bilstm", (2.0 * T * (4.0 * H * H * 4 + B * (H + H + 4 * H) * 4 * 2), T), (B, T, H))
    return out


def crop_descriptors(boxes, page_ids, page_hw, img_h, img_w):
    import numpy as np
    H, W = page_hw
    b = np.asarray(boxes, dtype=np.int64).reshape(-1, 4)
    pg = np.asarray(page_ids, dtype=np.int64).reshape(-1)
    a_, b_ = np.maximum(0, b[:, 0]), np.maximum(0, b[:, 1])
    c_, d_ = np.minimum(W, b[:, 2]), np.minimum(H, b[:, 3])
    c_ = np.where(c_ < 0, np.maximum(W + c_, 0), c_)
    d_ = np.where(d_ < 0, np.maximum(H + d_, 0), d_)
    keep = (c_ > a_) & (d_ > b_)
    a_, b_, c_, d_, pg = a_[keep], b_[keep], c_[keep], d_[keep], pg[keep]
    h, w = d_ - b_, c_ - a_
    scale = np.minimum(img_h / np.maximum(h, 1), img_w / np.maximum(w, 1))
    nw = np.maximum(1, np.rint(w * scale).astype(np.int64))
    nh = np.maximum(1, np.rint(h * scale).astype(np.int64))
    yy = np.maximum(0, np.minimum((img_h - nh) // 2, img_h - nh))
    desc = np.stack([pg, a_, b_, c_, d_, nw, nh, yy], axis=1).astype(np.int32) if len(pg) else np.zeros((0, 8), dtype=np.int32)
    return desc, keep


def _crop_descriptors_loop(boxes, page_ids, page_hw, img_h, img_w):
    import numpy as np
    H, W = page_hw
    desc, keep = [], []
    for (x0, y0, x1, y1), pg in zip(boxes, page_ids):
        a, b = max(0, int(x0)), max(0, int(y0))
        c, d = min(W, int(x1)), min(H, int(y1))
        if c < 0:
            c = max(W + c, 0)
        if d < 0:
            d = max(H + d, 0)
        if c <= a or d <= b:
            keep.append(False)
            continue
        h, w = d - b, c - a
        scale = min(img_h / max(h, 1), img_w / max(w, 1))
        nw, nh = max(1, int(round(w * scale))), max(1, int(round(h * scale)))
        yy = max(0, min((img_h - nh) // 2, img_h - nh))
        desc.append((pg, a, b, c, d, nw, nh, yy))
        keep.append(True)
    return np.asarray(desc, dtype=np.int32).reshape(-1, 8), np.asarray(keep, dtype=bool)


def crop_resize_pad(pages_u8, desc_host, img_h, img_w, desc_dev=None):
    _need_cuda(pages_u8, desc_dev)
    N, H, W, C = pages_u8.shape
    assert C == 3 and pages_u8.dtype == torch.uint8 and pages_u8.is_contiguous()
    hp = None
    if desc_host is not None:
        desc_host = desc_host.astype("int32", copy=False)
        hp = desc_host.ctypes.data
    M = len(desc_host) if desc_host is not None else int(desc_dev.shape[0])
    if desc_dev is None:
        desc_dev = torch.from_numpy(desc_host).to(pages_u8.device)
    else:
        assert desc_dev.dtype == torch.int32 and desc_dev.is_contiguous() and desc_dev.shape == (M, 8)
        desc_dev.record_stream(torch.cuda.current_stream())
    out = torch.empty((M, img_h, img_w, 3), dtype=torch.uint8, device=pages_u8.device)
    nat.check(nat.lib().msocr_crop_resize_pad(pages_u8.data_ptr(), N, H, W, desc_dev.data_ptr(), hp, M, img_h, img_w,
                                              out.data_ptr(), _stream()), "crop_resize_pad")
    return out
```

### manuscript_ocr_amd/recognizers/_trba/net.py

```python
import ctypes

import numpy as np
import os

import torch

from ... import _native as nat
from ... import ops
from ...detectors._east.net import BN_EPS, pack_stem_weight, stem_view, to_khwc


def _fold(sd, conv_key, bn_key):
    w = sd[conv_key + ".weight"].float()
    gamma, beta = sd[bn_key + ".weight"].float(), sd[bn_key + ".bias"].float()
    mean, var = sd[bn_key + ".running_mean"].float(), sd[bn_key + ".running_var"].float()
    s = gamma / torch.sqrt(var + BN_EPS)
    return w * s.view(-1, 1, 1, 1), beta - mean * s


def _gate_interleave(w_t, H):
    K = w_t.shape[0]
    return w_t.reshape(K, 4, H).permute(0, 2, 1).contiguous()


HOIST_CTX = os.environ.get("MSOCR_BEAM_HOIST", "1") != "0"

LAYER_SPEC = (("layer1", 1, 2), ("layer2", 2, 1), ("layer3", 5, 2), ("layer4", 3, 1))


class TrbaNet:
    def __init__(self, state_dict, num_classes, hidden=256, dtype=torch.float32, device="cuda", split=None):
        if hidden % 64 or not 64 <= hidden <= 512:
            raise ValueError(f"hidden_size must be a multiple of 64 between 64 and 512 for the HIP recurrent / attention kernels, got {hidden}")
        if num_classes > 512:
            raise ValueError(f"charsets above 512 tokens are not supported by the decoder kernels, got {num_classes}")
        self.dtype, self.device = dtype, torch.device(device)
        self.V, self.Hd = num_classes, hidden
        dev, sd = self.device, state_dict
        P = {}
        self.cpad = 4 if dtype == torch.float32 else 8
        self.cin_pad = 16 if dtype == torch.float32 else 32
        w, b = _fold(sd, "cnn.conv0.0", "cnn.conv0.1")
        P["stem"] = (pack_stem_weight(w, self.cin_pad, self.cpad).to(dtype).to(dev), b.to(dev))
        w, b = _fold(sd, "cnn.conv0.3", "cnn.conv0.4")
        P["conv0b"] = (to_khwc(w, dtype, dev, split), b.to(dev))
        for lname, blocks, stride in LAYER_SPEC:
            for i in range(blocks):
                p = f"cnn.{lname}.{i}."
                for j in (1, 2):
                    w, b = _fold(sd, p + f"conv{j}", p + f"bn{j}")
                    P[f"{lname}.{i}.conv{j}"] = (to_khwc(w, dtype, dev, split), b.to(dev))
                P[f"{lname}.{i}.se"] = (sd[p + "se.fc.0.weight"].float().contiguous().to(dev),
                                        sd[p + "se.fc.2.weight"].float().contiguous().to(dev))
                if p + "downsample.0.weight" in sd:
                    w, b = _fold(sd, p + "downsample.0", p + "downsample.1")
                    P[f"{lname}.{i}.down"] = (to_khwc(w, dtype, dev, split), b.to(dev))
        w, b = _fold(sd, "cnn.conv_out.0", "cnn.conv_out.1")
        P["out0"] = (to_khwc(w, dtype, dev, split), b.to(dev))
        w, b = _fold(sd, "cnn.conv_out.3", "cnn.conv_out.4")
        P["out1"] = (to_khwc(w, dtype, dev, split), b.to(dev))
        self.P = P
        H = hidden
        self.rnn = []
        for l in (0, 1):
            p = f"enc_rnn.{l}."
            w_ih = torch.cat([sd[p + "rnn.weight_ih_l0"], sd[p + "rnn.weight_ih_l0_reverse"]]).float()
            b = torch.cat([sd[p + "rnn.bias_ih_l0"] + sd[p + "rnn.bias_hh_l0"],
                           sd[p + "rnn.bias_ih_l0_reverse"] + sd[p + "rnn.bias_hh_l0_reverse"]]).float()
            whh_t = torch.stack([_gate_interleave(sd[p + "rnn.weight_hh_l0"].float().t(), H),
                                 _gate_interleave(sd[p + "rnn.weight_hh_l0_reverse"].float().t(), H)])
            whh_p = None
            if (ops.SPLIT_BF16X3 if split is None else split) and dtype == torch.float32 and H == 256:
                n = nat.lib().msocr_attn_pack_split_elems(4 * H)
                packed = torch.empty((2, n), dtype=torch.int16)
                wt = whh_t.contiguous()
                for d in (0, 1):
                    nat.check(nat.lib().msocr_attn_pack_split_host(wt[d].data_ptr(), 4 * H, 1, packed[d].data_ptr()), "attn_pack_split_host")
                whh_p = packed.to(dev)
            self.rnn.append({
                "w_ih": w_ih.view(8 * H, 1, 1, -1).contiguous().to(dev), "b": b.contiguous().to(dev),
                "whh_t": whh_t.contiguous().to(dev), "whh_p": whh_p,
                "lin_w": sd[p + "linear.weight"].float().view(H, 1, 1, 2 * H).contiguous().to(dev),
                "lin_b": sd[p + "linear.bias"].float().contiguous().to(dev),
            })
        a = "attn.attention_cell."
        w_ih = sd[a + "rnn.weight_ih"].float()
        self.att = {
            "i2h_w": sd[a + "i2h.weight"].float().view(H, 1, 1, H).contiguous().to(dev),
            "h2h_wt": sd[a + "h2h.weight"].float().t().contiguous().to(dev),
            "h2h_b": sd[a + "h2h.bias"].float().contiguous().to(dev),
            "score_w": sd[a + "score.weight"].float().view(H).contiguous().to(dev),
            "wih_ctx_t": _gate_interleave(w_ih[:, :H].t(), H).to(dev),
            "wih_tok": _gate_interleave(w_ih[:, H:].t(), H).to(dev),
            "whh_t": _gate_interleave(sd[a + "rnn.weight_hh"].float().t(), H).to(dev),
            "b_gates": _gate_interleave((sd[a + "rnn.bias_ih"] + sd[a + "rnn.bias_hh"]).float().view(1, 4 * H), H).view(H, 4).contiguous().to(dev),
            "gen_wt": sd["attn.generator.weight"].float().t().contiguous().to(dev),
            "gen_b": sd["attn.generator.bias"].float().contiguous().to(dev),
        }
        self.att["wih_ctx_rows"] = ops.attach_split(w_ih[:, :H].reshape(4, H, H).permute(1, 0, 2).reshape(4 * H, 1, 1, H).contiguous().to(dev),
                                                    split)
        aw = nat.AttnWeights()
        for k in ("h2h_wt", "h2h_b", "score_w", "wih_ctx_t", "wih_tok", "whh_t", "b_gates", "gen_wt", "gen_b"):
            setattr(aw, k, self.att[k].data_ptr())
        self._aw = aw
        self._asw = None
        if (ops.SPLIT_BF16X3 if split is None else split) and dtype == torch.float32 and H == 256 and self.V <= 256:
            asw = nat.AttnSplitWeights()
            for src, dst, n, gi in (("h2h_wt", "h2h_p", H, 0), ("whh_t", "whh_p", 4 * H, 1), ("gen_wt", "gen_p", self.V, 0)):
                wt = self.att[src].cpu().contiguous()
                packed = torch.empty((nat.lib().msocr_attn_pack_split_elems(n),), dtype=torch.int16)
                nat.check(nat.lib().msocr_attn_pack_split_host(wt.data_ptr(), n, gi, packed.data_ptr()), "attn_pack_split_host")
                self.att[dst] = packed.to(dev)
                setattr(asw, dst, self.att[dst].data_ptr())
            self._asw = asw

    def _se_block(self, x, lname, i, stride):
        P = self.P
        w1, b1 = P[f"{lname}.{i}.conv1"]
        w2, b2 = P[f"{lname}.{i}.conv2"]
        o = ops.conv2d(x, w1, b1, stride=(stride, stride), pad=(1, 1), relu=True)
        o = ops.conv2d(o, w2, b2, pad=(1, 1))
        key = f"{lname}.{i}.down"
        idt = ops.conv2d(x, *P[key], stride=(stride, stride)) if key in P else x
        s1, s2 = P[f"{lname}.{i}.se"]
        return ops.se_residual(o, idt, s1, s2)

    def cnn(self, canvases_u8):
        B, h, w, _ = canvases_u8.shape
        x = ops.normalize_u8(canvases_u8, 1, 1, h + 2, w + 4, 1, self.dtype, cpad=self.cpad)
        ws, bs = self.P["stem"]
        x = ops.conv2d(stem_view(x, self.cin_pad), ws, bs, (1, 1), (0, 0), True, out_hw=(h, w), alg_k=27)
        x = ops.conv2d(x, *self.P["conv0b"], pad=(1, 1), relu=True, pool2=True)
        for lname, blocks, stride in LAYER_SPEC:
            for i in range(blocks):
                x = self._se_block(x, lname, i, stride if i == 0 else 1)
        x = ops.conv2d(x, *self.P["out0"], stride=(2, 1), pad=(0, 1), relu=True)
        return ops.conv2d(x, *self.P["out1"], relu=True)

    def _gemm(self, x2d, w, b):
        M, K = x2d.shape
        return ops.conv2d(x2d.view(1, M, 1, K), w, b).view(M, w.shape[0])

    def encode(self, canvases_u8):
        f = self.cnn(canvases_u8)
        B, Hf, T, C = f.shape
        seq = ops.mean_over_h(f)
        H = self.Hd
        for l in (0, 1):
            r = self.rnn[l]
            xproj = self._gemm(seq.view(B * T, -1), r["w_ih"], r["b"])
            hcat = ops.bilstm_recurrent(xproj, r["whh_t"], B, T, H, r["whh_p"])
            seq = self._gemm(hcat.view(B * T, 2 * H), r["lin_w"], r["lin_b"]).view(B, T, H)
        proj = self._gemm(seq.view(B * T, H), self.att["i2h_w"], None).view(B, T, H)
        return seq, proj

    def greedy(self, batch_H, proj_H, max_len, sos_id, eos_id, blank_id):
        B, T, H = batch_H.shape
        steps = max_len + 1
        logits = torch.empty((B, steps, self.V), dtype=torch.float32, device=self.device)
        ids = torch.empty((B, steps), dtype=torch.int32, device=self.device)
        blank = -1 if blank_id is None else blank_id
        fast = H == 256 and self.V <= 256 and T <= 48 and getattr(self, "_asw", None) is not None
        if fast and HOIST_CTX and os.environ.get("MSOCR_GREEDY_MFMA", "1") != "0":
            ctxg = self._gemm(batch_H.reshape(B * T, H), self.att["wih_ctx_rows"], None)
            nat.check(nat.lib().msocr_attn_greedy_hoisted(batch_H.data_ptr(), proj_H.data_ptr(), ctxg.data_ptr(), ctypes.byref(self._aw),
                                                          ctypes.byref(self._asw), B, T, H, self.V, steps, sos_id, eos_id, blank,
                                                          logits.data_ptr(), ids.data_ptr(), ops._stream()), "attn_greedy_hoisted")
        else:
            nat.check(nat.lib().msocr_attn_greedy(batch_H.data_ptr(), proj_H.data_ptr(), ctypes.byref(self._aw), B, T, H, self.V, steps,
                                                  sos_id, eos_id, blank, logits.data_ptr(), ids.data_ptr(), ops._stream()), "attn_greedy")
        return logits, ids

    def beam(self, batch_H, proj_H, max_len, beam_size, alpha, temperature, sos_id, eos_id, blank_id, chunks=None):
        B, T, H = batch_H.shape
        steps = max_len
        nbytes = nat.lib().msocr_attn_beam_workspace_bytes(B, steps, beam_size, self.V)
        ws = torch.empty((nbytes,), dtype=torch.uint8, device=self.device)
        fin = torch.empty((B,), dtype=torch.int32, device=self.device)
        lp = None
        if alpha > 0:
            key = (float(alpha), steps)
            if not hasattr(self, "_lp_cache"):
                self._lp_cache = {}
            if key not in self._lp_cache:
                self._lp_cache[key] = torch.tensor([((5.0 + (t + 1)) ** alpha) / (6.0 ** alpha) for t in range(steps)],
                                                   dtype=torch.float32).to(self.device)
                torch.cuda.synchronize()
            lp = self._lp_cache[key]
        if not 1 <= beam_size <= 16 or (beam_size * H > 4096 and not (H == 256 and beam_size <= 8)):
            raise ValueError(f"beam_size {beam_size} with hidden_size {H}: the decoder kernels take beam_size <= 16 and beam_size x hidden_size <= 4096")
        fast = H == 256 and self.V <= 256 and T <= 48 and beam_size <= 8
        hoist = HOIST_CTX and fast and os.environ.get("MSOCR_BEAM_MFMA", "1") != "0"
        if hoist:
            ctxg = self._gemm(batch_H.reshape(B * T, H), self.att["wih_ctx_rows"], None)
        e = ops._prof_begin()
        tail = (B, T, H, self.V, steps, beam_size, lp.data_ptr() if lp is not None else None, float(temperature), sos_id, eos_id,
                -1 if blank_id is None else blank_id, fin.data_ptr(), ws.data_ptr(),
                chunks[0].data_ptr() if chunks else None, chunks[1].data_ptr() if chunks else None,
                chunks[2].data_ptr() if chunks else None, ops._stream())
        if hoist:
            asw = self._asw if os.environ.get("MSOCR_BEAM_SPLIT", "1") != "0" else None
            nat.check(nat.lib().msocr_attn_beam_hoisted(batch_H.data_ptr(), proj_H.data_ptr(), ctxg.data_ptr(), ctypes.byref(self._aw),
                                                        ctypes.byref(asw) if asw is not None else None, *tail), "attn_beam_hoisted")
        else:
            nat.check(nat.lib().msocr_attn_beam(batch_H.data_ptr(), proj_H.data_ptr(), ctypes.byref(self._aw), *tail), "attn_beam")
        V, R = self.V, B * beam_size
        per_step = 4.0 * (2 * B * T * H + 4 * H * (H + V) + 4 * H * H + H * V + H * H + R * (4 * H + V))
        ops._prof_end(e, "attn_beam", (per_step, steps), (B, T, beam_size))
        return ws, fin, lp

    def beam_finalize(self, ws, B, steps, beam_size, trun_dev):
        logits = torch.empty((B, steps, self.V), dtype=torch.float32, device=self.device)
        ids = torch.empty((B, steps), dtype=torch.int32, device=self.device)
        nat.check(nat.lib().msocr_attn_beam_finalize(ws.data_ptr(), B, self.V, steps, beam_size, trun_dev.data_ptr(), logits.data_ptr(),
                                                     ids.data_ptr(), ops._stream()), "attn_beam_finalize")
        return logits, ids


def trba_cnn_macs(h, w):
    macs = h * w * 64 * 27 + h * w * 128 * 64 * 9
    hh, ww, cin = h // 2, w // 2, 128
    for (lname, blocks, stride), planes in zip(LAYER_SPEC, (256, 256, 512, 512)):
        for i in range(blocks):
            s = stride if i == 0 else 1
            h2, w2 = (hh + 2 - 3) // s + 1, (ww + 2 - 3) // s + 1
            macs += h2 * w2 * planes * cin * 9 + h2 * w2 * planes * planes * 9
            if s != 1 or cin != planes:
                macs += h2 * w2 * planes * cin
            macs += 2 * planes * (planes // 16)
            hh, ww, cin = h2, w2, planes
    h3, w3 = (hh - 2) // 2 + 1, (ww + 2 - 2) + 1
    macs += h3 * w3 * 512 * 512 * 4
    macs += (h3 - 1) * (w3 - 1) * 512 * 512 * 4
    return macs
```

Measured before the change: 79.42.

## Chain TRBA SE-block Winograd convs through Winograd domain with fused SE tail

Adds two HIP kernels. The first runs the output transform of conv1 and writes the input transform for conv2 straight from LDS. The second fuses conv2's output transform with the squeeze-excite pooling, gating, residual add and ReLU, and also emits the next block's Winograd input tiles. The TRBA backbone plans runs of consecutive SE blocks and carves workspace regions out of a shared arena so intermediate spatial maps do not round-trip through global memory. This cuts kernel launches and HBM traffic, at the cost of the SE tail using one block per image, which may limit parallelism for small batches, and of more complex workspace bookkeeping.

```diff
diff --git a/include/msocr.h b/include/msocr.h
--- a/include/msocr.h
+++ b/include/msocr.h
@@ -43,6 +43,11 @@
 int msocr_winograd_gemm(const msocr_conv_desc* d, int form, int split, const void* u, void* workspace, void* stream);
 int msocr_winograd_output_transform(const msocr_conv_desc* d, int form, const void* workspace, const float* bias, const void* residual,
                                     void* out, void* stream);
+
+int msocr_winograd_chain(int N, int H, int W, int C, int form_out, int form_in, const void* mw, const float* bias, int relu, void* v,
+                         void* stream);
+int msocr_winograd_se_tail(int N, int H, int W, int C, int form_out, int form_next, const void* mw, const float* bias,
+                           const void* identity, const float* w1, const float* w2, float* gate, void* out, void* v_next, void* stream);
 
 int msocr_split_bf16x3_host(const float* w_host, int64_t n, uint16_t* planes_out_host);
 int msocr_split_bf16x3_ktile_host(const float* w_host, int64_t nbatch, int64_t rows, int64_t k, uint16_t* planes_out_host);
diff --git a/manuscript_ocr_amd/_native.py b/manuscript_ocr_amd/_native.py
--- a/manuscript_ocr_amd/_native.py
+++ b/manuscript_ocr_amd/_native.py
@@ -46,6 +46,8 @@
     "msocr_winograd_input_transform": (c_i32, [ctypes.POINTER(ConvDesc), c_i32, c_vp, c_vp, c_vp]),
     "msocr_winograd_gemm": (c_i32, [ctypes.POINTER(ConvDesc), c_i32, c_i32, c_vp, c_vp, c_vp]),
     "msocr_winograd_output_transform": (c_i32, [ctypes.POINTER(ConvDesc), c_i32, c_vp, c_vp, c_vp, c_vp, c_vp]),
+    "msocr_winograd_chain": (c_i32, [c_i32, c_i32, c_i32, c_i32, c_i32, c_i32, c_vp, c_vp, c_i32, c_vp, c_vp]),
+    "msocr_winograd_se_tail": (c_i32, [c_i32, c_i32, c_i32, c_i32, c_i32, c_i32, c_vp, c_vp, c_vp, c_vp, c_vp, c_vp, c_vp, c_vp, c_vp]),
     "msocr_winograd_fused64_workspace_bytes": (c_i64, [ctypes.POINTER(ConvDesc)]),
     "msocr_conv3x3_winograd_fused64": (c_i32, [ctypes.POINTER(ConvDesc), c_i32, c_vp, c_vp, c_vp, c_vp, c_vp, c_vp, c_vp]),
     "msocr_winograd_fused64_gemm_output": (c_i32, [ctypes.POINTER(ConvDesc), c_i32, c_vp, c_vp, c_vp, c_vp, c_vp, c_vp]),
diff --git a/manuscript_ocr_amd/csrc/trba_chain.hip b/manuscript_ocr_amd/csrc/trba_chain.hip
--- /dev/null
+++ b/manuscript_ocr_amd/csrc/trba_chain.hip
@@ -0,0 +1,276 @@
+#include <hip/hip_runtime.h>
+#include <math.h>
+#include <stdint.h>
+
+#include "internal.h"
+#include "msocr.h"
+#include "wino_transforms.h"
+
+#define MSOCR_LAUNCH(...) do { (void)hipGetLastError(); hipLaunchKernelGGL(__VA_ARGS__); } while (0)
+
+__device__ __forceinline__ float chain_sigmoidf(float x) { return 1.0f / (1.0f + expf(-x)); }
+__device__ __forceinline__ float chain_wave_sum(float v) {
+#pragma unroll
+  for (int o = 32; o > 0; o >>= 1) v += __shfl_xor(v, o);
+  return v;
+}
+
+static const int kChainTile[3][2] = {{2, 2}, {4, 2}, {4, 4}};
+
+static WinoGeom chain_geom(int N, int H, int W, int form) {
+  WinoGeom g;
+  g.N = N; g.H = H; g.W = W;
+  g.TH = (H + kChainTile[form][0] - 1) / kChainTile[form][0];
+  g.TW = (W + kChainTile[form][1] - 1) / kChainTile[form][1];
+  g.Mt = (long)N * g.TH * g.TW;
+  return g;
+}
+
+template <int MH, int MW>
+__device__ __forceinline__ void chain_input_from_lds(const float* map, int CS, const WinoGeom& g, int th, int tw, int c4, float* o,
+                                                     long plane) {
+  const int h0 = MH * th - 1, w0 = MW * tw - 1;
+  wino_input_tile<MH, MW>(
+      [&](int i, int j) {
+        const int hi = h0 + i, wi = w0 + j;
+        const bool ok = (unsigned)hi < (unsigned)g.H && (unsigned)wi < (unsigned)g.W;
+        return ok ? *reinterpret_cast<const f32x4*>(map + ((long)hi * g.W + wi) * CS + c4) : (f32x4){0.f, 0.f, 0.f, 0.f};
+      },
+      [&](int p, f32x4 v) { *reinterpret_cast<f32x4*>(o + p * plane) = v; });
+}
+
+template <int MH1, int MW1, int MH2, int MW2>
+__global__ __launch_bounds__(256) void wino_chain_kernel(const float* __restrict__ Mw1, int C, WinoGeom g1, WinoGeom g2, int NC, int CS,
+                                                         const float* __restrict__ bias, int relu, float* __restrict__ V2) {
+  extern __shared__ __attribute__((aligned(16))) float map[];
+  const int nsl = C / CS;
+  const int slice = blockIdx.x % nsl, grp = blockIdx.x / nsl;
+  const int n0 = grp * NC, nc = min(NC, g1.N - n0), c0 = slice * CS, q4 = CS / 4;
+  const int HW = g1.H * g1.W;
+  const int T1 = g1.TH * g1.TW, T2 = g2.TH * g2.TW;
+  {
+    const long plane = g1.Mt * (long)C;
+    for (int it = threadIdx.x; it < nc * T1 * q4; it += 256) {
+      const int q = it % q4, tl = it / q4, cl = tl / T1, tt = tl - cl * T1;
+      const int th = tt / g1.TW, tw = tt - th * g1.TW;
+      const int c4 = 4 * q;
+      const float* mp = Mw1 + ((long)(n0 + cl) * T1 + tt) * C + c0 + c4;
+      f32x4 b = {0.f, 0.f, 0.f, 0.f};
+      if (bias) b = *reinterpret_cast<const f32x4*>(bias + c0 + c4);
+      float* m = map + (long)cl * HW * CS + c4;
+      wino_output_tile<MH1, MW1>(
+          [&](int p) { return *reinterpret_cast<const f32x4*>(mp + p * plane); }, g1.H - MH1 * th,
+          [&](int a, const f32x4* y) {
+            const int ho = MH1 * th + a;
+#pragma unroll
+            for (int j = 0; j < MW1; ++j) {
+              const int wo = MW1 * tw + j;
+              if (wo >= g1.W) continue;
+              f32x4 v = y[j] + b;
+              if (relu) {
+                v[0] = fmaxf(v[0], 0.f); v[1] = fmaxf(v[1], 0.f); v[2] = fmaxf(v[2], 0.f); v[3] = fmaxf(v[3], 0.f);
+              }
+              *reinterpret_cast<f32x4*>(m + ((long)ho * g1.W + wo) * CS) = v;
+            }
+          });
+    }
+  }
+  __syncthreads();
+  const long plane = g2.Mt * (long)C;
+  for (int it = threadIdx.x; it < nc * T2 * q4; it += 256) {
+    const int q = it % q4, tl = it / q4, cl = tl / T2, tt = tl - cl * T2;
+    const int th = tt / g2.TW, tw = tt - th * g2.TW;
+    chain_input_from_lds<MH2, MW2>(map + (long)cl * HW * CS, CS, g2, th, tw, 4 * q,
+                                   V2 + ((long)(n0 + cl) * T2 + tt) * C + c0 + 4 * q, plane);
+  }
+}
+
+template <int MH2, int MW2, int MHN, int MWN, int NT>
+__global__ __launch_bounds__(NT) void wino_se_tail_kernel(const float* __restrict__ Mw2, int C, WinoGeom g2, WinoGeom gn, int CS,
+                                                          const float* __restrict__ bias, const float* __restrict__ idt,
+                                                          const float* __restrict__ w1, const float* __restrict__ w2,
+                                                          float* __restrict__ gate_ws, float* __restrict__ out, float* __restrict__ Vn) {
+  constexpr int VNT = 1024;
+  extern __shared__ __attribute__((aligned(16))) float sm[];
+  const int n = blockIdx.x, tid = threadIdx.x;
+  const int HW = g2.H * g2.W, C4 = C / 4, PG = VNT / C4;
+  const bool in_lds = CS == C;
+  float* buf = sm;
+  float* part = buf + (long)HW * CS;
+  float* mean = part + PG * C;
+  float* hid = mean + C;
+  float* gate = hid + C / 16;
+  float* os = out + (long)n * HW * C;
+  float* y2 = in_lds ? buf : os;
+  {
+    const int T2 = g2.TH * g2.TW;
+    const long plane = g2.Mt * (long)C;
+    for (int it = tid; it < T2 * C4; it += NT) {
+      const int q = it % C4, tt = it / C4;
+      const int th = tt / g2.TW, tw = tt - th * g2.TW;
+      const int c = 4 * q;
+      const float* mp = Mw2 + ((long)n * T2 + tt) * C + c;
+      f32x4 b = {0.f, 0.f, 0.f, 0.f};
+      if (bias) b = *reinterpret_cast<const f32x4*>(bias + c);
+      wino_output_tile<MH2, MW2>(
+          [&](int p) { return *reinterpret_cast<const f32x4*>(mp + p * plane); }, g2.H - MH2 * th,
+          [&](int a, const f32x4* y) {
+            const int ho = MH2 * th + a;
+#pragma unroll
+            for (int j = 0; j < MW2; ++j) {
+              const int wo = MW2 * tw + j;
+              if (wo >= g2.W) continue;
+              *reinterpret_cast<f32x4*>(y2 + ((long)ho * g2.W + wo) * C + c) = y[j] + b;
+            }
+          });
+    }
+  }
+  __syncthreads();
+  for (int vt = tid; vt < VNT; vt += NT) {
+    const int cg = vt % C4, pg = vt / C4;
+    f32x4 s = {0.f, 0.f, 0.f, 0.f};
+    for (int p = pg; p < HW; p += PG) {
+      const f32x4 v = *reinterpret_cast<const f32x4*>(y2 + (long)p * C + cg * 4);
+      s[0] += v[0]; s[1] += v[1]; s[2] += v[2]; s[3] += v[3];
+    }
+    *reinterpret_cast<f32x4*>(&part[pg * C + cg * 4]) = s;
+  }
+  __syncthreads();
+  const float inv = 1.0f / (float)HW;
+  for (int c = tid; c < C; c += NT) {
+    float s = 0.f;
+    for (int g = 0; g < PG; ++g) s += part[g * C + c];
+    mean[c] = s * inv;
+  }
+  __syncthreads();
+  const int Cr = C / 16;
+  {
+    const int lane = tid & 63, wv = tid >> 6;
+    for (int j = wv; j < Cr; j += NT / 64) {
+      float a = 0.f;
+      for (int c = lane; c < C; c += 64) a = fmaf(w1[(long)j * C + c], mean[c], a);
+      a = chain_wave_sum(a);
+      if (lane == 0) hid[j] = fmaxf(a, 0.f);
+    }
+  }
+  __syncthreads();
+  for (int c = tid; c < C; c += NT) {
+    float a = 0.f;
+    for (int j = 0; j < Cr; ++j) a = fmaf(w2[(long)c * Cr + j], hid[j], a);
+    const float g = chain_sigmoidf(a);
+    gate[c] = g;
+    gate_ws[(long)n * C + c] = g;
+  }
+  __syncthreads();
+  const float* is = idt + (long)n * HW * C;
+  const int q4 = CS / 4;
+  for (int c0 = 0; c0 < C; c0 += CS) {
+    for (int it = tid; it < HW * q4; it += NT) {
+      const int q = it % q4, p = it / q4;
+      const long o = (long)p * C + c0 + 4 * q;
+      const f32x4 v = *reinterpret_cast<const f32x4*>(y2 + o), r = *reinterpret_cast<const f32x4*>(is + o);
+      const f32x4 g4 = *reinterpret_cast<const f32x4*>(&gate[c0 + 4 * q]);
+      f32x4 y;
+#pragma unroll
+      for (int e = 0; e < 4; ++e) y[e] = fmaxf(v[e] * g4[e] + r[e], 0.f);
+      *reinterpret_cast<f32x4*>(os + o) = y;
+      if constexpr (MHN > 0) *reinterpret_cast<f32x4*>(buf + (long)p * CS + 4 * q) = y;
+    }
+    if constexpr (MHN > 0) {
+      __syncthreads();
+      const int Tn = gn.TH * gn.TW;
+      const long plane = gn.Mt * (long)C;
+      for (int it = tid; it < Tn * q4; it += NT) {
+        const int q = it % q4, tt = it / q4;
+        const int th = tt / gn.TW, tw = tt - th * gn.TW;
+        chain_input_from_lds<MHN, MWN>(buf, CS, gn, th, tw, 4 * q, Vn + ((long)n * Tn + tt) * C + c0 + 4 * q, plane);
+      }
+      __syncthreads();
+    }
+  }
+}
+
+static bool chain_ok(int N, int H, int W, int C, int form) {
+  return N > 0 && H > 0 && W > 0 && C >= 64 && C <= 1024 && !(C & (C - 1)) && form >= MSOCR_WINO_2X2 && form <= MSOCR_WINO_4X4 &&
+         (long)N * H * W * C <= 0x3fffffffffffL;
+}
+
+static const long kLdsBudget = 108 * 1024;
+static const long kChainLds = 64 * 1024;
+
+static void chain_shape(int H, int W, int C, int form1, int* nc, int* cs) {
+  const int T1 = ((H + kChainTile[form1][0] - 1) / kChainTile[form1][0]) * ((W + kChainTile[form1][1] - 1) / kChainTile[form1][1]);
+  *cs = C < 64 ? C : 64;
+  while (*cs > 16 && (long)H * W * *cs * 4 > kChainLds) *cs >>= 1;
+  *nc = 256 / (T1 * (*cs / 4));
+  if (*nc < 1) *nc = 1;
+  while (*nc > 1 && (long)*nc * H * W * *cs * 4 > kChainLds) --*nc;
+}
+
+template <int F1>
+static void* chain_kernel_ptr(int form2) {
+  constexpr int MH1 = F1 == MSOCR_WINO_2X2 ? 2 : 4, MW1 = F1 == MSOCR_WINO_4X4 ? 4 : 2;
+  if (form2 == MSOCR_WINO_2X2) return (void*)wino_chain_kernel<MH1, MW1, 2, 2>;
+  if (form2 == MSOCR_WINO_4X2) return (void*)wino_chain_kernel<MH1, MW1, 4, 2>;
+  return (void*)wino_chain_kernel<MH1, MW1, 4, 4>;
+}
+
+extern "C" int msocr_winograd_chain(int N, int H, int W, int C, int form_out, int form_in, const void* mw, const float* bias, int relu,
+                                    void* v, void* stream) {
+  if (!chain_ok(N, H, W, C, form_out) || !chain_ok(N, H, W, C, form_in) || !mw || !v) return MSOCR_E_ARG;
+  if ((((uintptr_t)mw | (uintptr_t)v | (uintptr_t)bias) & 15)) return MSOCR_E_ARG;
+  int nc, cs;
+  chain_shape(H, W, C, form_out, &nc, &cs);
+  const long lds = (long)nc * H * W * cs * 4;
+  if (lds > kLdsBudget) return MSOCR_E_ARG;
+  const long nblk = (long)((N + nc - 1) / nc) * (C / cs);
+  if (nblk > 0x7fffffffL) return MSOCR_E_ARG;
+  const WinoGeom g1 = chain_geom(N, H, W, form_out), g2 = chain_geom(N, H, W, form_in);
+  const void* kern = form_out == MSOCR_WINO_2X2 ? chain_kernel_ptr<MSOCR_WINO_2X2>(form_in)
+                     : form_out == MSOCR_WINO_4X2 ? chain_kernel_ptr<MSOCR_WINO_4X2>(form_in)
+                                                  : chain_kernel_ptr<MSOCR_WINO_4X4>(form_in);
+  if (hipFuncSetAttribute(kern, hipFuncAttributeMaxDynamicSharedMemorySize, (int)lds) != hipSuccess) return MSOCR_E_LAUNCH;
+  const float* mwf = (const float*)mw;
+  float* vf = (float*)v;
+  void* args[] = {&mwf, &C, (void*)&g1, (void*)&g2, &nc, &cs, &bias, &relu, &vf};
+  (void)hipGetLastError();
+  if (hipLaunchKernel(kern, dim3((unsigned)nblk), dim3(256), args, (size_t)lds, (hipStream_t)stream) != hipSuccess) return MSOCR_E_LAUNCH;
+  return hipGetLastError() == hipSuccess ? MSOCR_OK : MSOCR_E_LAUNCH;
+}
+
+constexpr int kTailNT = 512;
+
+template <int F2>
+static void* tail_kernel_ptr(int form_next) {
+  constexpr int MH2 = F2 == MSOCR_WINO_2X2 ? 2 : 4, MW2 = F2 == MSOCR_WINO_4X4 ? 4 : 2;
+  if (form_next == MSOCR_WINO_2X2) return (void*)wino_se_tail_kernel<MH2, MW2, 2, 2, kTailNT>;
+  if (form_next == MSOCR_WINO_4X2) return (void*)wino_se_tail_kernel<MH2, MW2, 4, 2, kTailNT>;
+  if (form_next == MSOCR_WINO_4X4) return (void*)wino_se_tail_kernel<MH2, MW2, 4, 4, kTailNT>;
+  return (void*)wino_se_tail_kernel<MH2, MW2, 0, 0, kTailNT>;
+}
+
+extern "C" int msocr_winograd_se_tail(int N, int H, int W, int C, int form_out, int form_next, const void* mw, const float* bias,
+                                      const void* identity, const float* w1, const float* w2, float* gate, void* out, void* v_next,
+                                      void* stream) {
+  if (!chain_ok(N, H, W, C, form_out) || !mw || !identity || !w1 || !w2 || !gate || !out) return MSOCR_E_ARG;
+  if (form_next >= 0 && (!chain_ok(N, H, W, C, form_next) || !v_next)) return MSOCR_E_ARG;
+  if ((((uintptr_t)mw | (uintptr_t)bias | (uintptr_t)identity | (uintptr_t)out | (uintptr_t)v_next) & 15)) return MSOCR_E_ARG;
+  const long HW = (long)H * W;
+  int cs = C;
+  while (cs > 4 && HW * cs * 4 > kLdsBudget) cs >>= 1;
+  if (HW * cs * 4 > kLdsBudget) return MSOCR_E_ARG;
+  const long lds = (HW * cs + (long)(1024 / (C / 4)) * C + 2 * C + C / 16) * 4;
+  const WinoGeom g2 = chain_geom(N, H, W, form_out), gn = chain_geom(N, H, W, form_next >= 0 ? form_next : form_out);
+  const void* kern = form_out == MSOCR_WINO_2X2 ? tail_kernel_ptr<MSOCR_WINO_2X2>(form_next)
+                     : form_out == MSOCR_WINO_4X2 ? tail_kernel_ptr<MSOCR_WINO_4X2>(form_next)
+                                                  : tail_kernel_ptr<MSOCR_WINO_4X4>(form_next);
+  if (hipFuncSetAttribute(kern, hipFuncAttributeMaxDynamicSharedMemorySize, (int)lds) != hipSuccess) return MSOCR_E_LAUNCH;
+  const float* mwf = (const float*)mw;
+  const float* idf = (const float*)identity;
+  float* of = (float*)out;
+  float* vf = (float*)v_next;
+  void* args[] = {&mwf, &C, (void*)&g2, (void*)&gn, &cs, &bias, &idf, &w1, &w2, &gate, &of, &vf};
+  (void)hipGetLastError();
+  if (hipLaunchKernel(kern, dim3((unsigned)N), dim3(kTailNT), args, (size_t)lds, (hipStream_t)stream) != hipSuccess) return MSOCR_E_LAUNCH;
+  return hipGetLastError() == hipSuccess ? MSOCR_OK : MSOCR_E_LAUNCH;
+}
diff --git a/manuscript_ocr_amd/csrc/wino_transforms.h b/manuscript_ocr_amd/csrc/wino_transforms.h
--- /dev/null
+++ b/manuscript_ocr_amd/csrc/wino_transforms.h
@@ -0,0 +1,128 @@
+#ifndef MSOCR_WINO_TRANSFORMS_H
+#define MSOCR_WINO_TRANSFORMS_H
+#include <hip/hip_runtime.h>
+
+typedef float f32x4 __attribute__((ext_vector_type(4)));
+
+template <int M> __device__ void wino_bt1(const f32x4 d[M + 2], f32x4 r[M + 2]);
+template <int M> __device__ void wino_at1(const f32x4 m[M + 2], f32x4 y[M]);
+
+template <> __device__ __forceinline__ void wino_bt1<2>(const f32x4 d[4], f32x4 r[4]) {
+  r[0] = d[0] - d[2];
+  r[1] = d[1] + d[2];
+  r[2] = d[2] - d[1];
+  r[3] = d[1] - d[3];
+}
+template <> __device__ __forceinline__ void wino_at1<2>(const f32x4 m[4], f32x4 y[2]) {
+  y[0] = (m[0] + m[1]) + m[2];
+  y[1] = (m[1] - m[2]) - m[3];
+}
+
+__device__ __forceinline__ void wino44_bt(const f32x4 d[6], f32x4 r[6]) {
+  constexpr float k97_36 = 97.0f / 36.0f, k4_9 = 4.0f / 9.0f, k9_4 = 2.25f, k3_2 = 1.5f, k2_3 = 2.0f / 3.0f;
+#pragma unroll
+  for (int e = 0; e < 4; ++e) {
+    r[0][e] = fmaf(-k97_36, d[2][e], d[0][e]) + d[4][e];
+    r[5][e] = fmaf(-k97_36, d[3][e], d[1][e]) + d[5][e];
+    const float e1 = fmaf(-k4_9, d[2][e], d[4][e]), o1 = fmaf(k3_2, d[3][e], -k2_3 * d[1][e]);
+    const float e2 = fmaf(-k9_4, d[2][e], d[4][e]), o2 = fmaf(k2_3, d[3][e], -k3_2 * d[1][e]);
+    r[1][e] = e1 + o1; r[2][e] = e1 - o1;
+    r[3][e] = e2 + o2; r[4][e] = e2 - o2;
+  }
+}
+__device__ __forceinline__ void wino44_at(const f32x4 m[6], f32x4 y[4]) {
+  constexpr float k3_2 = 1.5f, k2_3 = 2.0f / 3.0f, k9_4 = 2.25f, k4_9 = 4.0f / 9.0f, k27_8 = 3.375f, k8_27 = 8.0f / 27.0f;
+#pragma unroll
+  for (int e = 0; e < 4; ++e) {
+    const float p12 = m[1][e] + m[2][e], d12 = m[1][e] - m[2][e], p34 = m[3][e] + m[4][e], d34 = m[3][e] - m[4][e];
+    y[0][e] = (m[0][e] + p12) + p34;
+    y[1][e] = fmaf(k3_2, d12, k2_3 * d34);
+    y[2][e] = fmaf(k9_4, p12, k4_9 * p34);
+    y[3][e] = fmaf(k27_8, d12, k8_27 * d34) + m[5][e];
+  }
+}
+template <> __device__ __forceinline__ void wino_bt1<4>(const f32x4 d[6], f32x4 r[6]) { wino44_bt(d, r); }
+template <> __device__ __forceinline__ void wino_at1<4>(const f32x4 m[6], f32x4 y[4]) { wino44_at(m, y); }
+
+
+struct WinoGeom {
+  int N, H, W;
+  int TH, TW;
+  long Mt;
+};
+
+template <int MH, int MW, class Load, class Store>
+__device__ __forceinline__ void wino_input_tile(Load ld, Store st) {
+  constexpr int PH = MH + 2, PW = MW + 2;
+  constexpr bool w_first = MH == 4;
+  f32x4 q[PH][PW];
+#pragma unroll
+  for (int i = 0; i < PH; ++i) {
+    f32x4 d[PW];
+#pragma unroll
+    for (int j = 0; j < PW; ++j) d[j] = ld(i, j);
+    if constexpr (w_first) {
+      wino_bt1<MW>(d, q[i]);
+    } else {
+#pragma unroll
+      for (int j = 0; j < PW; ++j) q[i][j] = d[j];
+    }
+  }
+  if constexpr (w_first) {
+#pragma unroll
+    for (int j = 0; j < PW; ++j) {
+      f32x4 col[PH], v[PH];
+#pragma unroll
+      for (int i = 0; i < PH; ++i) col[i] = q[i][j];
+      wino_bt1<MH>(col, v);
+#pragma unroll
+      for (int i = 0; i < PH; ++i) st(i * PW + j, v[i]);
+    }
+  } else {
+#pragma unroll
+    for (int i = 0; i < PH; ++i) {
+      f32x4 row[PW], v[PW];
+#pragma unroll
+      for (int j = 0; j < PW; ++j) {
+        f32x4 col[PH], hv[PH];
+#pragma unroll
+        for (int k = 0; k < PH; ++k) col[k] = q[k][j];
+        wino_bt1<MH>(col, hv);
+        row[j] = hv[i];
+      }
+      wino_bt1<MW>(row, v);
+#pragma unroll
+      for (int j = 0; j < PW; ++j) st(i * PW + j, v[j]);
+    }
+  }
+}
+
+template <int MH, int MW, class Load, class Emit>
+__device__ __forceinline__ void wino_output_tile(Load ldm, int rows, Emit emit) {
+  constexpr int PH = MH + 2, PW = MW + 2;
+  f32x4 mt[PH][PW];
+  if constexpr (MH == 2) {
+#pragma unroll
+    for (int i = 0; i < PH; ++i)
+#pragma unroll
+      for (int j = 0; j < PW; ++j) mt[i][j] = ldm(i * PW + j);
+  }
+  f32x4 s[MH][PW];
+#pragma unroll
+  for (int j = 0; j < PW; ++j) {
+    f32x4 m[PH], y[MH];
+#pragma unroll
+    for (int i = 0; i < PH; ++i) m[i] = MH == 2 ? mt[i][j] : ldm(i * PW + j);
+    wino_at1<MH>(m, y);
+#pragma unroll
+    for (int a = 0; a < MH; ++a) s[a][j] = y[a];
+  }
+#pragma unroll
+  for (int a = 0; a < MH; ++a) {
+    if (a >= rows) continue;
+    f32x4 y[MW];
+    wino_at1<MW>(s[a], y);
+    emit(a, y);
+  }
+}
+#endif
diff --git a/manuscript_ocr_amd/csrc/winograd.hip b/manuscript_ocr_amd/csrc/winograd.hip
--- a/manuscript_ocr_amd/csrc/winograd.hip
+++ b/manuscript_ocr_amd/csrc/winograd.hip
@@ -3,62 +3,12 @@
 
 #include "internal.h"
 #include "msocr.h"
+#include "wino_transforms.h"
 
 #define MSOCR_LAUNCH(...) do { (void)hipGetLastError(); hipLaunchKernelGGL(__VA_ARGS__); } while (0)
-
-typedef float f32x4 __attribute__((ext_vector_type(4)));
-
-template <int M> __device__ void wino_bt1(const f32x4 d[M + 2], f32x4 r[M + 2]);
-template <int M> __device__ void wino_at1(const f32x4 m[M + 2], f32x4 y[M]);
-
-template <> __device__ __forceinline__ void wino_bt1<2>(const f32x4 d[4], f32x4 r[4]) {
-  r[0] = d[0] - d[2];
-  r[1] = d[1] + d[2];
-  r[2] = d[2] - d[1];
-  r[3] = d[1] - d[3];
-}
-template <> __device__ __forceinline__ void wino_at1<2>(const f32x4 m[4], f32x4 y[2]) {
-  y[0] = (m[0] + m[1]) + m[2];
-  y[1] = (m[1] - m[2]) - m[3];
-}
-
-__device__ __forceinline__ void wino44_bt(const f32x4 d[6], f32x4 r[6]) {
-  constexpr float k97_36 = 97.0f / 36.0f, k4_9 = 4.0f / 9.0f, k9_4 = 2.25f, k3_2 = 1.5f, k2_3 = 2.0f / 3.0f;
-#pragma unroll
-  for (int e = 0; e < 4; ++e) {
-    r[0][e] = fmaf(-k97_36, d[2][e], d[0][e]) + d[4][e];
-    r[5][e] = fmaf(-k97_36, d[3][e], d[1][e]) + d[5][e];
-    const float e1 = fmaf(-k4_9, d[2][e], d[4][e]), o1 = fmaf(k3_2, d[3][e], -k2_3 * d[1][e]);
-    const float e2 = fmaf(-k9_4, d[2][e], d[4][e]), o2 = fmaf(k2_3, d[3][e], -k3_2 * d[1][e]);
-    r[1][e] = e1 + o1; r[2][e] = e1 - o1;
-    r[3][e] = e2 + o2; r[4][e] = e2 - o2;
-  }
-}
-__device__ __forceinline__ void wino44_at(const f32x4 m[6], f32x4 y[4]) {
-  constexpr float k3_2 = 1.5f, k2_3 = 2.0f / 3.0f, k9_4 = 2.25f, k4_9 = 4.0f / 9.0f, k27_8 = 3.375f, k8_27 = 8.0f / 27.0f;
-#pragma unroll
-  for (int e = 0; e < 4; ++e) {
-    const float p12 = m[1][e] + m[2][e], d12 = m[1][e] - m[2][e], p34 = m[3][e] + m[4][e], d34 = m[3][e] - m[4][e];
-    y[0][e] = (m[0][e] + p12) + p34;
-    y[1][e] = fmaf(k3_2, d12, k2_3 * d34);
-    y[2][e] = fmaf(k9_4, p12, k4_9 * p34);
-    y[3][e] = fmaf(k27_8, d12, k8_27 * d34) + m[5][e];
-  }
-}
-template <> __device__ __forceinline__ void wino_bt1<4>(const f32x4 d[6], f32x4 r[6]) { wino44_bt(d, r); }
-template <> __device__ __forceinline__ void wino_at1<4>(const f32x4 m[6], f32x4 y[4]) { wino44_at(m, y); }
-
-
-struct WinoGeom {
-  int N, H, W;
-  int TH, TW;
-  long Mt;
-};
 
 template <int MH, int MW>
 __device__ __forceinline__ void wino_input_body(const float* in, long sN, long sH, long sW, int C, WinoGeom g, float* V) {
-  constexpr int PH = MH + 2, PW = MW + 2;
-  constexpr bool w_first = MH == 4;
   const int cch = C >> 2;
   const long gid = (long)blockIdx.x * 256 + threadIdx.x;
   const long t = gid / cch;
@@ -70,61 +20,21 @@
   const int n = (int)(r / g.TH);
   const int h0 = MH * th - 1, w0 = MW * tw - 1;
   const float* base = in + (long)n * sN + c;
-  f32x4 q[PH][PW];
-#pragma unroll
-  for (int i = 0; i < PH; ++i) {
-    const int hi = h0 + i;
-    const bool okh = (unsigned)hi < (unsigned)g.H;
-    f32x4 d[PW];
-#pragma unroll
-    for (int j = 0; j < PW; ++j) {
-      const int wi = w0 + j;
-      const bool ok = okh && (unsigned)wi < (unsigned)g.W;
-      const f32x4 v = *reinterpret_cast<const f32x4*>(ok ? base + (long)hi * sH + (long)wi * sW : base);
-      d[j] = ok ? v : (f32x4){0.f, 0.f, 0.f, 0.f};
-    }
-    if constexpr (w_first) {
-      wino_bt1<MW>(d, q[i]);
-    } else {
-#pragma unroll
-      for (int j = 0; j < PW; ++j) q[i][j] = d[j];
-    }
-  }
   const long plane = g.Mt * (long)C;
   float* o = V + t * (long)C + c;
-  if constexpr (w_first) {
-#pragma unroll
-    for (int j = 0; j < PW; ++j) {
-      f32x4 col[PH], v[PH];
-#pragma unroll
-      for (int i = 0; i < PH; ++i) col[i] = q[i][j];
-      wino_bt1<MH>(col, v);
-#pragma unroll
-      for (int i = 0; i < PH; ++i) *reinterpret_cast<f32x4*>(o + (i * PW + j) * plane) = v[i];
-    }
-  } else {
-#pragma unroll
-    for (int i = 0; i < PH; ++i) {
-      f32x4 row[PW], v[PW];
-#pragma unroll
-      for (int j = 0; j < PW; ++j) {
-        f32x4 col[PH], hv[PH];
-#pragma unroll
-        for (int k = 0; k < PH; ++k) col[k] = q[k][j];
-        wino_bt1<MH>(col, hv);
-        row[j] = hv[i];
-      }
-      wino_bt1<MW>(row, v);
-#pragma unroll
-      for (int j = 0; j < PW; ++j) *reinterpret_cast<f32x4*>(o + (i * PW + j) * plane) = v[j];
-    }
-  }
+  wino_input_tile<MH, MW>(
+      [&](int i, int j) {
+        const int hi = h0 + i, wi = w0 + j;
+        const bool ok = (unsigned)hi < (unsigned)g.H && (unsigned)wi < (unsigned)g.W;
+        const f32x4 v = *reinterpret_cast<const f32x4*>(ok ? base + (long)hi * sH + (long)wi * sW : base);
+        return ok ? v : (f32x4){0.f, 0.f, 0.f, 0.f};
+      },
+      [&](int p, f32x4 v) { *reinterpret_cast<f32x4*>(o + p * plane) = v; });
 }
 
 template <int MH, int MW>
 __device__ __forceinline__ void wino_output_body(const float* Mw, int Cout, WinoGeom g, const float* bias, const float* res, long res_ld,
                                                  int relu, float* out, long out_ld) {
-  constexpr int PH = MH + 2, PW = MW + 2;
   const int cch = Cout >> 2;
   const long gid = (long)blockIdx.x * 256 + threadIdx.x;
   const long t = gid / cch;
@@ -136,44 +46,25 @@
   const int n = (int)(r / g.TH);
   const long plane = g.Mt * (long)Cout;
   const float* mp = Mw + t * (long)Cout + c;
-  f32x4 mt[PH][PW];
-  if constexpr (MH == 2) {
-#pragma unroll
-    for (int i = 0; i < PH; ++i)
-#pragma unroll
-      for (int j = 0; j < PW; ++j) mt[i][j] = *reinterpret_cast<const f32x4*>(mp + (i * PW + j) * plane);
-  }
-  f32x4 s[MH][PW];
-#pragma unroll
-  for (int j = 0; j < PW; ++j) {
-    f32x4 m[PH], y[MH];
-#pragma unroll
-    for (int i = 0; i < PH; ++i) m[i] = MH == 2 ? mt[i][j] : *reinterpret_cast<const f32x4*>(mp + (i * PW + j) * plane);
-    wino_at1<MH>(m, y);
-#pragma unroll
-    for (int a = 0; a < MH; ++a) s[a][j] = y[a];
-  }
   f32x4 b = {0.f, 0.f, 0.f, 0.f};
   if (bias) b = *reinterpret_cast<const f32x4*>(bias + c);
-#pragma unroll
-  for (int a = 0; a < MH; ++a) {
-    const int ho = MH * th + a;
-    if (ho >= g.H) continue;
-    f32x4 y[MW];
-    wino_at1<MW>(s[a], y);
-#pragma unroll
-    for (int j = 0; j < MW; ++j) {
-      const int wo = MW * tw + j;
-      if (wo >= g.W) continue;
-      const long pix = ((long)n * g.H + ho) * g.W + wo;
-      f32x4 v = y[j] + b;
-      if (res) v += *reinterpret_cast<const f32x4*>(res + pix * res_ld + c);
-      if (relu) {
-        v[0] = fmaxf(v[0], 0.f); v[1] = fmaxf(v[1], 0.f); v[2] = fmaxf(v[2], 0.f); v[3] = fmaxf(v[3], 0.f);
-      }
-      *reinterpret_cast<f32x4*>(out + pix * out_ld + c) = v;
-    }
-  }
+  wino_output_tile<MH, MW>(
+      [&](int p) { return *reinterpret_cast<const f32x4*>(mp + p * plane); }, g.H - MH * th,
+      [&](int a, const f32x4* y) {
+        const int ho = MH * th + a;
+#pragma unroll
+        for (int j = 0; j < MW; ++j) {
+          const int wo = MW * tw + j;
+          if (wo >= g.W) continue;
+          const long pix = ((long)n * g.H + ho) * g.W + wo;
+          f32x4 v = y[j] + b;
+          if (res) v += *reinterpret_cast<const f32x4*>(res + pix * res_ld + c);
+          if (relu) {
+            v[0] = fmaxf(v[0], 0.f); v[1] = fmaxf(v[1], 0.f); v[2] = fmaxf(v[2], 0.f); v[3] = fmaxf(v[3], 0.f);
+          }
+          *reinterpret_cast<f32x4*>(out + pix * out_ld + c) = v;
+        }
+      });
 }
 
 #define WINO_TRANSFORM_KERNELS(PREFIX, MH, MW)                                                                                    \
diff --git a/manuscript_ocr_amd/ops.py b/manuscript_ocr_amd/ops.py
--- a/manuscript_ocr_amd/ops.py
+++ b/manuscript_ocr_amd/ops.py
@@ -56,6 +56,22 @@
 
 WINO_WS_LIMIT = int(os.environ.get("MSOCR_WINO_WS_LIMIT", str(1 << 30)))
 _WINO_ARENA = {}
+
+
+def wino_arena_take(nbytes, device):
+    buf = _wino_workspace(nbytes, device)
+    if not torch.cuda.is_current_stream_capturing():
+        _WINO_ARENA.pop((device.index, torch.cuda.current_stream().cuda_stream), None)
+    return buf
+
+
+def wino_arena_return(buf, device):
+    if torch.cuda.is_current_stream_capturing():
+        return
+    key = (device.index, torch.cuda.current_stream().cuda_stream)
+    cur = _WINO_ARENA.get(key)
+    if cur is None or cur.numel() < buf.numel():
+        _WINO_ARENA[key] = buf
 
 
 def _wino_workspace(nbytes, device):
@@ -212,6 +228,85 @@
     d.N = N
 
 
+def wino_choice(w, H, W):
+    u = getattr(w, "_msocr_wino", None)
+    if u is None:
+        return None
+    form, split = nat.WINO_2X2, False
+    if WINOGRAD_TALL and _tall_pays(H) and getattr(w, "_msocr_wino42", None) is not None:
+        form, u = nat.WINO_4X2, w._msocr_wino42
+        up = getattr(w, "_msocr_wino42_split", None)
+        if up is not None and SPLIT_BF16X3:
+            u, split = up, True
+        up44 = getattr(w, "_msocr_wino44_split", None)
+        if up44 is not None and SPLIT_BF16X3 and WINOGRAD_SQUARE and _square_pays(W):
+            form, u, split = nat.WINO_4X4, up44, True
+    return form, u, split
+
+
+def wino_tiles(form, H, W):
+    _, npts, (mh, mw) = WINO_FORMS[form]
+    return npts, (-(-H // mh)) * (-(-W // mw))
+
+
+def _wino_region_desc(N, H, W, Cin, Cout, x=None):
+    d = nat.ConvDesc()
+    d.dtype = nat.F32
+    d.N, d.H, d.W, d.Cin = N, H, W, Cin
+    d.in_sN, d.in_sH, d.in_sW = (x.stride(0), x.stride(1), x.stride(2)) if x is not None else (H * W * Cin, W * Cin, Cin)
+    d.KH, d.KW, d.stride_h, d.stride_w, d.pad_h, d.pad_w = 3, 3, 1, 1, 1, 1
+    d.Ho, d.Wo, d.Cout = H, W, Cout
+    d.out_ld = Cout
+    return d
+
+
+def winograd_input_region(x, Cout, form, region):
+    N, H, W, Cin = x.shape
+    d = _wino_region_desc(N, H, W, Cin, Cout, x)
+    npts, tiles = wino_tiles(form, H, W)
+    e = _prof_begin()
+    nat.check(nat.lib().msocr_winograd_input_transform(ctypes.byref(d), form, x.data_ptr(), region, _stream()),
+              f"msocr_winograd_input_transform {tuple(x.shape)}")
+    _prof_end(e, "wino_in", 4.0 * (N * H * W * Cin + npts * N * tiles * Cin), (N * tiles, Cin))
+
+
+def winograd_gemm_region(N, H, W, Cin, Cout, form, split, u, region):
+    d = _wino_region_desc(N, H, W, Cin, Cout)
+    npts, tiles = wino_tiles(form, H, W)
+    mt = N * tiles
+    e = _prof_begin()
+    nat.check(nat.lib().msocr_winograd_gemm(ctypes.byref(d), form, int(split), u.data_ptr(), region, _stream()),
+              f"msocr_winograd_gemm {(N, H, W, Cin, Cout)} form {form}")
+    io = 4.0 * (N * H * W * Cin + N * H * W * Cout + Cout * 9 * Cin)
+    _prof_end(e, "conv_gemm", (2.0 * N * H * W * Cout * 9 * Cin, 2.0 * npts * mt * Cin * Cout, io),
+              (N * H * W, Cout, 9 * Cin, WINO_FORMS[form][0] + ("_split" if split else "")))
+    return region + 4 * npts * mt * Cin
+
+
+def winograd_chain(mw, N, H, W, C, form_out, form_in, bias, v, relu=True):
+    p_out, t_out = wino_tiles(form_out, H, W)
+    p_in, t_in = wino_tiles(form_in, H, W)
+    e = _prof_begin()
+    nat.check(nat.lib().msocr_winograd_chain(N, H, W, C, form_out, form_in, mw, bias.data_ptr() if bias is not None else None,
+                                             int(relu), v, _stream()), f"msocr_winograd_chain {(N, H, W, C, form_out, form_in)}")
+    _prof_end(e, "wino_out", 4.0 * N * C * (p_out * t_out + p_in * t_in), (N * t_out, C))
+
+
+def winograd_se_tail(mw, N, H, W, C, form_out, bias, identity, w1, w2, out, form_next=-1, v_next=None):
+    _need_cuda(identity, w1, w2, out)
+    assert identity.shape == (N, H, W, C) and out.shape == (N, H, W, C) and identity.is_contiguous() and out.is_contiguous()
+    assert identity.dtype == torch.float32 and out.dtype == torch.float32 and w1.shape == (C // 16, C) and w2.shape == (C, C // 16)
+    gate = torch.empty((N, C), dtype=torch.float32, device=out.device)
+    p_out, t_out = wino_tiles(form_out, H, W)
+    vn = 0 if form_next < 0 else N * C * wino_tiles(form_next, H, W)[0] * wino_tiles(form_next, H, W)[1]
+    e = _prof_begin()
+    nat.check(nat.lib().msocr_winograd_se_tail(N, H, W, C, form_out, form_next, mw, bias.data_ptr() if bias is not None else None,
+                                               identity.data_ptr(), w1.data_ptr(), w2.data_ptr(), gate.data_ptr(), out.data_ptr(),
+                                               v_next, _stream()), f"msocr_winograd_se_tail {(N, H, W, C, form_out, form_next)}")
+    _prof_end(e, "se_residual", 4.0 * (p_out * N * t_out * C + 2 * N * H * W * C + vn), (N, H * W, C))
+    return gate
+
+
 def conv2d(x, w, bias, stride=(1, 1), pad=(0, 0), relu=False, residual=None, out=None, out_hw=None, alg_k=None, pool2=False):
     _need_cuda(x, w, bias, residual, out)
     N, H, W, Cin = x.shape
@@ -255,15 +350,7 @@
         u = w._msocr_wino42_fused if up is None else up
         _winograd(d, x, w, u, nat.WINO_4X2, up is not None, bias, residual, out, alg, fused=True, pool2=pool2)
     elif use_wino:
-        form, split = nat.WINO_2X2, False
-        if WINOGRAD_TALL and _tall_pays(H) and getattr(w, "_msocr_wino42", None) is not None:
-            form, u = nat.WINO_4X2, w._msocr_wino42
-            up = getattr(w, "_msocr_wino42_split", None)
-            if up is not None and SPLIT_BF16X3:
-                u, split = up, True
-            up44 = getattr(w, "_msocr_wino44_split", None)
-            if up44 is not None and SPLIT_BF16X3 and WINOGRAD_SQUARE and _square_pays(W):
-                form, u, split = nat.WINO_4X4, up44, True
+        form, u, split = wino_choice(w, H, W)
         _winograd(d, x, w, u, form, split, bias, residual, out, alg)
     else:
         wp = getattr(w, "_msocr_split", None)
diff --git a/manuscript_ocr_amd/recognizers/_trba/net.py b/manuscript_ocr_amd/recognizers/_trba/net.py
--- a/manuscript_ocr_amd/recognizers/_trba/net.py
+++ b/manuscript_ocr_amd/recognizers/_trba/net.py
@@ -26,6 +26,8 @@
 HOIST_CTX = os.environ.get("MSOCR_BEAM_HOIST", "1") != "0"
 
 LAYER_SPEC = (("layer1", 1, 2), ("layer2", 2, 1), ("layer3", 5, 2), ("layer4", 3, 1))
+
+TRBA_CHAIN = os.environ.get("MSOCR_TRBA_CHAIN", "1") != "0"
 
 
 class TrbaNet:
@@ -125,15 +127,105 @@
         s1, s2 = P[f"{lname}.{i}.se"]
         return ops.se_residual(o, idt, s1, s2)
 
+    def _chain_plan(self, lname, i, stride, H, W):
+        w1, b1 = self.P[f"{lname}.{i}.conv1"]
+        w2, b2 = self.P[f"{lname}.{i}.conv2"]
+        C = w1.shape[0]
+        Ho, Wo = (H - 1) // stride + 1, (W - 1) // stride + 1
+        c2 = ops.wino_choice(w2, Ho, Wo)
+        if c2 is None or w1.dtype != torch.float32 or C & (C - 1) or not 64 <= C <= 1024:
+            return None
+        c1 = ops.wino_choice(w1, H, W) if stride == 1 else None
+        return {"name": f"{lname}.{i}", "stride": stride, "H": H, "W": W, "Cin": w1.shape[3], "C": C, "Ho": Ho, "Wo": Wo,
+                "c1": c1, "c2": c2}
+
+    def _se_run(self, x, run):
+        N = x.shape[0]
+        P = self.P
+        need, v1 = 0, 0
+        for j, pl in enumerate(run):
+            pl["vin"] = j > 0
+            if pl["c1"] is not None:
+                npts, tiles = ops.wino_tiles(pl["c1"][0], pl["H"], pl["W"])
+                m1, s_m1 = v1 + 4 * npts * tiles * pl["Cin"], 4 * npts * tiles * pl["C"]
+                pl["v1"], end1 = v1, m1 + s_m1
+            else:
+                m1, end1 = 0, 0
+            npts, tiles = ops.wino_tiles(pl["c2"][0], pl["Ho"], pl["Wo"])
+            s_v2 = 4 * npts * tiles * pl["C"]
+            pl["v2"] = 0 if pl["c1"] is None or s_v2 <= m1 else end1
+            m2 = pl["v2"] + s_v2
+            need = max(need, end1, m2 + s_v2)
+            if j + 1 < len(run):
+                nx = run[j + 1]
+                npts, tiles = ops.wino_tiles(nx["c1"][0], nx["H"], nx["W"])
+                s_vn = 4 * npts * tiles * nx["Cin"]
+                v1 = 0 if s_vn <= m2 else m2 + s_v2
+                need = max(need, v1 + s_vn)
+        parts = min(N, -(-N * need // ops.WINO_WS_LIMIT))
+        per = -(-N // parts)
+        last = run[-1]
+        out = torch.empty((N, last["Ho"], last["Wo"], last["C"]), dtype=x.dtype, device=x.device)
+        ws = ops.wino_arena_take(per * need, x.device)
+        base = ws.data_ptr()
+        for n0 in range(0, N, per):
+            n1 = min(N, n0 + per)
+            nn = n1 - n0
+            xp = x[n0:n1]
+            for j, pl in enumerate(run):
+                w1, b1 = P[pl["name"] + ".conv1"]
+                w2, b2 = P[pl["name"] + ".conv2"]
+                s, H, W, Ho, Wo, C = pl["stride"], pl["H"], pl["W"], pl["Ho"], pl["Wo"], pl["C"]
+                f2, u2, sp2 = pl["c2"]
+                v2 = base + nn * pl["v2"]
+                if pl["c1"] is not None:
+                    f1, u1, sp1 = pl["c1"]
+                    v1 = base + nn * pl["v1"]
+                    if not pl["vin"]:
+                        ops.winograd_input_region(xp, C, f1, v1)
+                    mw1 = ops.winograd_gemm_region(nn, H, W, pl["Cin"], C, f1, sp1, u1, v1)
+                    ops.winograd_chain(mw1, nn, Ho, Wo, C, f1, f2, b1, v2, relu=True)
+                else:
+                    ops.winograd_input_region(ops.conv2d(xp, w1, b1, stride=(s, s), pad=(1, 1), relu=True), C, f2, v2)
+                mw2 = ops.winograd_gemm_region(nn, Ho, Wo, C, C, f2, sp2, u2, v2)
+                key = pl["name"] + ".down"
+                idt = ops.conv2d(xp, *P[key], stride=(s, s)) if key in P else xp
+                nxt = run[j + 1] if j + 1 < len(run) else None
+                o = out[n0:n1] if nxt is None else torch.empty((nn, Ho, Wo, C), dtype=x.dtype, device=x.device)
+                s1, s2 = P[pl["name"] + ".se"]
+                ops.winograd_se_tail(mw2, nn, Ho, Wo, C, f2, b2, idt, s1, s2, o,
+                                     form_next=nxt["c1"][0] if nxt else -1, v_next=base + nn * nxt["v1"] if nxt else None)
+                xp = o
+        ops.wino_arena_return(ws, x.device)
+        return out
+
+    def _se_layers(self, x):
+        blocks = [(lname, i, stride if i == 0 else 1) for lname, n, stride in LAYER_SPEC for i in range(n)]
+        k = 0
+        while k < len(blocks):
+            run = []
+            _, H, W, _ = x.shape
+            while TRBA_CHAIN and k + len(run) < len(blocks):
+                pl = self._chain_plan(*blocks[k + len(run)], H, W)
+                if pl is None or (run and pl["c1"] is None):
+                    break
+                run.append(pl)
+                H, W = pl["Ho"], pl["Wo"]
+            if run:
+                x = self._se_run(x, run)
+                k += len(run)
+            else:
+                x = self._se_block(x, *blocks[k])
+                k += 1
+        return x
+
     def cnn(self, canvases_u8):
         B, h, w, _ = canvases_u8.shape
         x = ops.normalize_u8(canvases_u8, 1, 1, h + 2, w + 4, 1, self.dtype, cpad=self.cpad)
         ws, bs = self.P["stem"]
         x = ops.conv2d(stem_view(x, self.cin_pad), ws, bs, (1, 1), (0, 0), True, out_hw=(h, w), alg_k=27)
         x = ops.conv2d(x, *self.P["conv0b"], pad=(1, 1), relu=True, pool2=True)
-        for lname, blocks, stride in LAYER_SPEC:
-            for i in range(blocks):
-                x = self._se_block(x, lname, i, stride if i == 0 else 1)
+        x = self._se_layers(x)
         x = ops.conv2d(x, *self.P["out0"], stride=(2, 1), pad=(0, 1), relu=True)
         return ops.conv2d(x, *self.P["out1"], relu=True)
 
```

Result: no change. 80.72 (median of 6 runs) (+1.6%).
